# CIAM-Group/ComputerVision_Codes

Measured on AMD Instinct MI355X. Metric: frames/sec spatial-extract + per-video TCN latency, Cholec80, 1/2/4/8 GPU, higher is better.
Workload: dtype bf16

## Files before the change

computervision_codes_amd/csrc/bottleneck_fused.hip:

```cpp
#include "mt4_common.h"

typedef __bf16 bf16x8_t __attribute__((ext_vector_type(8)));

namespace {

constexpr int TH = 8, TW = 14, NHALO = 160, NPX = 128;
constexpr int ROW_B = 128;
constexpr int XS_BYTES = NHALO * ROW_B;
constexpr int T2_BYTES = NPX * ROW_B;
constexpr int T1_BYTES = XS_BYTES + 2 * ROW_B;
constexpr int YS_BYTES = NPX * 256;

struct BneckK {
    const char* x;
    char* y;
    const char *w1, *w2, *w3, *wds;
    const float *b1, *b2, *b3, *bds;
    int B, H, W, tiles_h, tiles_w;
    int nt;
    char* y2;
    const char* wn;
    const float* bn;
    int H2, W2;
};

__device__ __forceinline__ f32x4 bias4(const float* b, int n) {
    const float4 t = *(const float4*)(b + n);
    return (f32x4){t.x, t.y, t.z, t.w};
}

__device__ __forceinline__ uint2 relu_pack4(f32x4 v) {
    uint2 o = make_uint2(pack_bf16x2(v[0], v[1]), pack_bf16x2(v[2], v[3]));
    asm("v_pk_max_i16 %0, %0, 0" : "+v"(o.x));
    asm("v_pk_max_i16 %0, %0, 0" : "+v"(o.y));
    return o;
}

__device__ __forceinline__ f32x4 mfma_bf16(uint4 wfrag, uint4 xfrag, f32x4 acc) {
    return __builtin_amdgcn_mfma_f32_16x16x32_bf16(__builtin_bit_cast(bf16x8_t, wfrag), __builtin_bit_cast(bf16x8_t, xfrag), acc, 0, 0, 0);
}

template <int CIN, bool DS, bool NEXT = false>
__global__ __launch_bounds__(256, 2) void bottleneck64_fused_kernel(const BneckK a) {
    static_assert(!NEXT || !DS, "the following conv rides behind an identity block");
    constexpr int KC = CIN / 64;
    constexpr int NXS = KC > 1 ? 2 : 1;
    static_assert(DS ? CIN == 64 : CIN == 256, "layer1.0 (64 channels in, downsample branch) or layer1.1+ (256 in, identity)");
    extern __shared__ __attribute__((aligned(16))) char smem[];
    char* const xs = smem;
    char* const t2 = smem + NXS * XS_BYTES;
    char* const t1 = t2 + T2_BYTES;
    char* const ys = DS ? t1 : xs;

    const int tid = threadIdx.x;
    const int lane = tid & 63, wave = tid >> 6;
    const int r16 = lane & 15, q = lane >> 4;

    int bid = blockIdx.x;
    {
        const int nb = gridDim.x;
        const int q8 = nb >> 3, r8 = nb & 7;
        const int xcd = bid & 7, local = bid >> 3;
        bid = (xcd < r8 ? xcd * (q8 + 1) : r8 * (q8 + 1) + (xcd - r8) * q8) + local;
    }
    const int tpi = a.tiles_h * a.tiles_w;
    const int img = bid / tpi;
    const int trem = bid - img * tpi;
    const int th = trem / a.tiles_w;
    const int h0 = th * TH, w0 = (trem - th * a.tiles_w) * TW;
    const char* const ximg = a.x + (long long)img * a.H * a.W * (CIN * 2);
    char* const yimg = NEXT ? a.y + (long long)img * a.H2 * a.W2 * 512 : a.y + (long long)img * a.H * a.W * 512;

    const int ld_row = tid >> 3, ld_chunk = tid & 7;
    int xoff[5];
#pragma unroll
    for (int i = 0; i < 5; ++i) {
        const int hp = ld_row + 32 * i;
        const int h = h0 - 1 + (hp >> 4), w = w0 - 1 + (hp & 15);
        xoff[i] = ((unsigned)h < (unsigned)a.H && (unsigned)w < (unsigned)a.W) ? (h * a.W + w) * (CIN * 2) + ld_chunk * 16 : -1;
    }
    auto load_chunk = [&](int kc, uint4 (&stg)[5]) {
#pragma unroll
        for (int i = 0; i < 5; ++i) {
            stg[i] = make_uint4(0, 0, 0, 0);
            if (xoff[i] >= 0) stg[i] = *(const uint4*)(ximg + xoff[i] + kc * 128);
        }
    };
    auto store_chunk = [&](int buf, const uint4 (&stg)[5]) {
#pragma unroll
        for (int i = 0; i < 5; ++i) {
            const int hp = ld_row + 32 * i;
            *(uint4*)(xs + buf * XS_BYTES + hp * ROW_B + ((ld_chunk ^ (hp & 7)) << 4)) = stg[i];
        }
    };
    uint4 stg0[5], stg1[5];
    load_chunk(0, stg0);
    if constexpr (KC > 1) load_chunk(1, stg1);

    const int ch1 = wave * 16;
    uint4 wf1[KC * 2];
    {
        const char* wr = a.w1 + (wave * (KC * 2) * 64 + lane) * 16;
#pragma unroll
        for (int s = 0; s < KC * 2; ++s) wf1[s] = *(const uint4*)(wr + s * 1024);
    }
    f32x4 acc1[10];
    {
        const f32x4 b4 = bias4(a.b1, ch1 + q * 4);
#pragma unroll
        for (int i = 0; i < 10; ++i) acc1[i] = b4;
    }
    const int sw0 = (q ^ (r16 & 7)) << 4, sw1 = ((4 + q) ^ (r16 & 7)) << 4;
    uint2 res[DS ? 1 : 4][DS ? 1 : 8];
    const int res_off = (r16 + 1) * ROW_B + (((2 * wave + (q >> 1)) ^ ((r16 + 1) & 7)) << 4) + (q & 1) * 8;
#pragma unroll
    for (int kc = 0; kc < KC; ++kc) {
        if (kc & 1) store_chunk(1, stg1); else store_chunk(0, stg0);
        if (kc + 2 < KC) { if (kc & 1) load_chunk(kc + 2, stg1); else load_chunk(kc + 2, stg0); }
        __syncthreads();
        const char* sb = xs + (kc & 1) * XS_BYTES + r16 * ROW_B;
        uint4 fx[2][10];
#pragma unroll
        for (int kk = 0; kk < 2; ++kk)
#pragma unroll
            for (int i = 0; i < 10; ++i) fx[kk][i] = *(const uint4*)(sb + i * 16 * ROW_B + (kk ? sw1 : sw0));
        if constexpr (!DS) {
#pragma unroll
            for (int j = 0; j < 8; ++j) res[kc][j] = *(const uint2*)(xs + (kc & 1) * XS_BYTES + (j + 1) * (16 * ROW_B) + res_off);
        }
        asm volatile("" ::: "memory");
#pragma unroll
        for (int kk = 0; kk < 2; ++kk)
#pragma unroll
            for (int i = 0; i < 10; ++i) acc1[i] = mfma_bf16(wf1[kc * 2 + kk], fx[kk][i], acc1[i]);
    }
    uint4 wf2[18];
    {
        const char* wr = a.w2 + (wave * 18 * 64 + lane) * 16;
#pragma unroll
        for (int s = 0; s < 18; ++s) wf2[s] = *(const uint4*)(wr + s * 1024);
    }
    const int cb1 = (ch1 + q * 4) * 2;
    {
        const int wr_off = r16 * ROW_B + (((cb1 >> 4) ^ (r16 & 7)) << 4) + (cb1 & 8);
        const int w = w0 - 1 + r16;
#pragma unroll
        for (int i = 0; i < 10; ++i) {
            const int h = h0 - 1 + i;
            const bool in = (unsigned)h < (unsigned)a.H && (unsigned)w < (unsigned)a.W;
            uint2 o = make_uint2(0, 0);
            if (in) o = relu_pack4(acc1[i]);
            *(uint2*)(t1 + i * (16 * ROW_B) + wr_off) = o;
        }
    }
    __syncthreads();

    f32x4 acc2[8];
    {
        const f32x4 b4 = bias4(a.b2, ch1 + q * 4);
#pragma unroll
        for (int j = 0; j < 8; ++j) acc2[j] = b4;
    }
    int toff[3][2];
#pragma unroll
    for (int kw = 0; kw < 3; ++kw)
#pragma unroll
        for (int kk = 0; kk < 2; ++kk) toff[kw][kk] = (r16 + kw) * ROW_B + (((kk * 4 + q) ^ ((r16 + kw) & 7)) << 4);
#pragma unroll
    for (int hr = 0; hr < 10; ++hr) {
        uint4 fr[3][2];
#pragma unroll
        for (int kw = 0; kw < 3; ++kw)
#pragma unroll
            for (int kk = 0; kk < 2; ++kk) fr[kw][kk] = *(const uint4*)(t1 + hr * (16 * ROW_B) + toff[kw][kk]);
        asm volatile("" ::: "memory");
#pragma unroll
        for (int kh = 0; kh < 3; ++kh) {
            const int ty = hr - kh;
            if (ty >= 0 && ty < 8) {
#pragma unroll
                for (int kw = 0; kw < 3; ++kw)
#pragma unroll
                    for (int kk = 0; kk < 2; ++kk) acc2[ty] = mfma_bf16(wf2[(kh * 3 + kw) * 2 + kk], fr[kw][kk], acc2[ty]);
            }
        }
    }
    uint4 wf3[4][2];
    uint4 wfd[DS ? 4 : 1][2];
#pragma unroll
    for (int i = 0; i < 4; ++i) {
        const char* wr = a.w3 + ((4 * i + wave) * 2 * 64 + lane) * 16;
        wf3[i][0] = *(const uint4*)wr;
        wf3[i][1] = *(const uint4*)(wr + 1024);
        if constexpr (DS) {
            const char* wd = a.wds + ((4 * i + wave) * 2 * 64 + lane) * 16;
            wfd[i][0] = *(const uint4*)wd;
            wfd[i][1] = *(const uint4*)(wd + 1024);
        }
    }
    {
        const int wr_off = r16 * ROW_B + (((cb1 >> 4) ^ (r16 & 7)) << 4) + (cb1 & 8);
#pragma unroll
        for (int j = 0; j < 8; ++j) {
            const uint2 o = relu_pack4(acc2[j]);
            *(uint2*)(t2 + j * (16 * ROW_B) + wr_off) = o;
        }
    }
    __syncthreads();

    uint4 fx3[8][2];
#pragma unroll
    for (int j = 0; j < 8; ++j) {
        fx3[j][0] = *(const uint4*)(t2 + j * (16 * ROW_B) + r16 * ROW_B + sw0);
        fx3[j][1] = *(const uint4*)(t2 + j * (16 * ROW_B) + r16 * ROW_B + sw1);
    }
    const int st_tx = tid >> 4, st_chunk = tid & 15;
    uint4 wfn[NEXT ? 2 : 1][NEXT ? 8 : 1];
#pragma unroll
    for (int pass = 0; pass < 2; ++pass) {
        char* const ysp = NEXT ? xs + pass * YS_BYTES : ys;
        if (pass && !NEXT) __syncthreads();
#pragma unroll
        for (int ii = 0; ii < 2; ++ii) {
            const int i = pass * 2 + ii;
            const int ct = 4 * i + wave;
            f32x4 acc3[8];
            {
                const f32x4 b4 = bias4(a.b3, ct * 16 + q * 4);
#pragma unroll
                for (int j = 0; j < 8; ++j) acc3[j] = b4;
            }
#pragma unroll
            for (int kk = 0; kk < 2; ++kk)
#pragma unroll
                for (int j = 0; j < 8; ++j) acc3[j] = mfma_bf16(wf3[i][kk], fx3[j][kk], acc3[j]);
            if constexpr (DS) {
                const f32x4 bd4 = bias4(a.bds, ct * 16 + q * 4);
#pragma unroll
                for (int j = 0; j < 8; ++j) {
                    f32x4 accd = bd4;
#pragma unroll
                    for (int kk = 0; kk < 2; ++kk) accd = mfma_bf16(wfd[i][kk], *(const uint4*)(xs + (j + 1) * (16 * ROW_B) + toff[1][kk]), accd);
#pragma unroll
                    for (int e = 0; e < 4; ++e) acc3[j][e] += bf16_to_f32(f32_to_bf16(accd[e]));
                }
            } else {
#pragma unroll
                for (int j = 0; j < 8; ++j) {
                    acc3[j][0] += __uint_as_float(res[i][j].x << 16);
                    acc3[j][1] += __uint_as_float(res[i][j].x & 0xffff0000u);
                    acc3[j][2] += __uint_as_float(res[i][j].y << 16);
                    acc3[j][3] += __uint_as_float(res[i][j].y & 0xffff0000u);
                }
            }
            const int cbyte = ((ct - 8 * pass) * 16 + q * 4) * 2;
            const int wr_off = r16 * 256 + (((cbyte >> 4) ^ r16) << 4) + (cbyte & 8);
#pragma unroll
            for (int j = 0; j < 8; ++j) {
                const uint2 o = relu_pack4(acc3[j]);
                *(uint2*)(ysp + j * (16 * 256) + wr_off) = o;
            }
        }
        if constexpr (NEXT) {
            if (pass == 1) {
#pragma unroll
                for (int c = 0; c < 2; ++c)
#pragma unroll
                    for (int ks = 0; ks < 8; ++ks) wfn[c][ks] = *(const uint4*)(a.wn + (((2 * wave + c) * 8 + ks) * 64 + lane) * 16);
            }
        }
        __syncthreads();
        {
            const int w = w0 + st_tx;
            const int rd_off = st_tx * 256 + ((st_chunk ^ st_tx) << 4);
            if constexpr (NEXT) {
                if (st_tx < TW && w < a.W && !(st_tx & 1)) {
                    const uint4 v0 = *(const uint4*)(ysp + rd_off), v1 = *(const uint4*)(ysp + 2 * (16 * 256) + rd_off);
                    const uint4 v2 = *(const uint4*)(ysp + 4 * (16 * 256) + rd_off), v3 = *(const uint4*)(ysp + 6 * (16 * 256) + rd_off);
                    char* const yp = yimg + (unsigned)(((h0 >> 1) * a.W2 + (w >> 1)) * 512 + pass * 256 + st_chunk * 16);
                    const int rows = a.H - h0;
                    *(uint4*)yp = v0;
                    if (rows > 2) *(uint4*)(yp + a.W2 * 512) = v1;
                    if (rows > 4) *(uint4*)(yp + 2 * a.W2 * 512) = v2;
                    if (rows > 6) *(uint4*)(yp + 3 * a.W2 * 512) = v3;
                }
            } else if (st_tx < TW && w < a.W) {
                uint4 v[8];
#pragma unroll
                for (int ty = 0; ty < 8; ++ty) v[ty] = *(const uint4*)(ysp + ty * (16 * 256) + rd_off);
                asm volatile("" ::: "memory");
#pragma unroll
                for (int ty = 0; ty < 8; ++ty) {
                    if (h0 + ty < a.H) {
                        typedef unsigned u32x4 __attribute__((ext_vector_type(4)));
                        char* yp = yimg + (unsigned)((h0 + ty) * a.W * 512) + (unsigned)(w * 512 + pass * 256 + st_chunk * 16);
                        if (a.nt) __builtin_nontemporal_store((u32x4){v[ty].x, v[ty].y, v[ty].z, v[ty].w}, (u32x4*)yp);
                        else *(uint4*)yp = v[ty];
                    }
                }
            }
        }
    }
    if constexpr (NEXT) {
        f32x4 acc4[2][8];
#pragma unroll
        for (int c = 0; c < 2; ++c) {
            const f32x4 b4 = bias4(a.bn, (2 * wave + c) * 16 + q * 4);
#pragma unroll
            for (int j = 0; j < 8; ++j) acc4[c][j] = b4;
        }
#pragma unroll
        for (int ks = 0; ks < 8; ++ks) {
            uint4 fy[8];
            const char* yb = xs + (ks >> 2) * YS_BYTES + r16 * 256 + ((((ks & 3) * 4 + q) ^ r16) << 4);
#pragma unroll
            for (int j = 0; j < 8; ++j) fy[j] = *(const uint4*)(yb + j * (16 * 256));
            asm volatile("" ::: "memory");
#pragma unroll
            for (int c = 0; c < 2; ++c)
#pragma unroll
                for (int j = 0; j < 8; ++j) acc4[c][j] = mfma_bf16(wfn[c][ks], fy[j], acc4[c][j]);
        }
        __syncthreads();
#pragma unroll
        for (int c = 0; c < 2; ++c) {
            const int cbyte = ((2 * wave + c) * 16 + q * 4) * 2;
            const int wr_off = r16 * 256 + (((cbyte >> 4) ^ r16) << 4) + (cbyte & 8);
#pragma unroll
            for (int j = 0; j < 8; ++j) *(uint2*)(xs + j * (16 * 256) + wr_off) = relu_pack4(acc4[c][j]);
        }
        __syncthreads();
        const int w = w0 + st_tx;
        if (st_tx < TW && w < a.W) {
            const int rd_off = st_tx * 256 + ((st_chunk ^ st_tx) << 4);
            char* const y2img = a.y2 + (long long)img * a.H * a.W * 256;
            uint4 v[8];
#pragma unroll
            for (int ty = 0; ty < 8; ++ty) v[ty] = *(const uint4*)(xs + ty * (16 * 256) + rd_off);
            asm volatile("" ::: "memory");
#pragma unroll
            for (int ty = 0; ty < 8; ++ty) {
                if (h0 + ty < a.H) {
                    typedef unsigned u32x4 __attribute__((ext_vector_type(4)));
                    char* yp = y2img + (unsigned)(((h0 + ty) * a.W + w) * 256 + st_chunk * 16);
                    if (a.nt) __builtin_nontemporal_store((u32x4){v[ty].x, v[ty].y, v[ty].z, v[ty].w}, (u32x4*)yp);
                    else *(uint4*)yp = v[ty];
                }
            }
        }
    }
}

template <int CIN, bool DS, bool NEXT = false>
int launch(const BneckK& a, hipStream_t stream) {
    constexpr int NXS = CIN > 64 ? 2 : 1;
    constexpr int LDS = NXS * XS_BYTES + T2_BYTES + (DS ? YS_BYTES : T1_BYTES);
    static_assert(LDS <= 80 * 1024, "two workgroups per CU");
    static_assert(!NEXT || LDS >= 2 * YS_BYTES, "both output passes stay in LDS");
    auto fn = bottleneck64_fused_kernel<CIN, DS, NEXT>;
    MT4_RAISE_LDS(fn);
    const long long nblk = (long long)a.B * a.tiles_h * a.tiles_w;
    hipLaunchKernelGGL(fn, dim3((unsigned)nblk), dim3(256), LDS, stream, a);
    return mt4_check_launch();
}

}

__global__ void bneck_pack_kernel(const u16* __restrict__ w, uint4* __restrict__ out, int ctiles, int ksteps, int row_elems) {
    const int i = blockIdx.x * blockDim.x + threadIdx.x;
    if (i >= ctiles * ksteps * 64) return;
    const int lane = i & 63, fs = i >> 6;
    const int step = fs % ksteps, tile = fs / ksteps;
    out[i] = *(const uint4*)(w + (long long)(tile * 16 + (lane & 15)) * row_elems + step * 32 + (lane >> 4) * 8);
}

static inline long long bneck_frag_bytes(int Cin, bool ds) { return ((long long)4 * (Cin / 32) + 4 * 18 + 16 * 2 + (ds ? 16 * (Cin / 32) : 0)) * 1024; }

extern "C" int64_t mt4_bottleneck_packed_bytes(int32_t Cin, int32_t has_downsample) {
    if (!((has_downsample && Cin == 64) || (!has_downsample && Cin == 256))) return MT4_EUNSUPPORTED;
    return bneck_frag_bytes(Cin, has_downsample != 0);
}

extern "C" int mt4_bottleneck_pack_bf16(const void* w1, const void* w2, const void* w3, const void* wds, int32_t Cin, void* out, void* stream) {
    mt4_clear_error();
    if (!w1 || !w2 || !w3 || !out) return MT4_EINVAL;
    if (!((wds && Cin == 64) || (!wds && Cin == 256))) return MT4_EUNSUPPORTED;
    if (((uintptr_t)w1 | (uintptr_t)w2 | (uintptr_t)w3 | (uintptr_t)wds | (uintptr_t)out) & 15) return MT4_EALIGN;
    hipStream_t s = (hipStream_t)stream;
    const int k1 = Cin / 32;
    char* o = (char*)out;
    const int r1 = (int)mt4_conv_packed_k(Cin, 1, 1, MT4_BF16), r2 = (int)mt4_conv_packed_k(64, 3, 3, MT4_BF16), r3 = (int)mt4_conv_packed_k(64, 1, 1, MT4_BF16);
    auto go = [&](const void* w, int ctiles, int ksteps, int row_elems) {
        const int n = ctiles * ksteps * 64;
        hipLaunchKernelGGL(bneck_pack_kernel, dim3((n + 255) / 256), dim3(256), 0, s, (const u16*)w, (uint4*)o, ctiles, ksteps, row_elems);
        o += (long long)n * 16;
    };
    go(w1, 4, k1, r1);
    go(w2, 4, 18, r2);
    go(w3, 16, 2, r3);
    if (wds) go(wds, 16, k1, r1);
    return mt4_check_launch();
}

extern "C" int mt4_bottleneck_fused_bf16(const void* x, void* y, const void* w_frag, const float* b1, const float* b2, const float* b3, const float* bds,
                                         int32_t B, int32_t H, int32_t W, int32_t Cin, int32_t mid, void* stream) {
    mt4_clear_error();
    if (!x || !y || !w_frag || !b1 || !b2 || !b3 || B <= 0 || H <= 0 || W <= 0) return MT4_EINVAL;
    const bool ds = bds != nullptr;
    if (mid != 64 || !((ds && Cin == 64) || (!ds && Cin == 256))) return MT4_EUNSUPPORTED;
    if (((uintptr_t)x | (uintptr_t)y | (uintptr_t)w_frag | (uintptr_t)b1 | (uintptr_t)b2 | (uintptr_t)b3 | (uintptr_t)bds) & 15) return MT4_EALIGN;
    if ((long long)H * W * 512 > 0x7fffffffLL) return MT4_EUNSUPPORTED;
    BneckK a;
    a.x = (const char*)x; a.y = (char*)y;
    const int k1 = Cin / 32;
    a.w1 = (const char*)w_frag;
    a.w2 = a.w1 + (long long)4 * k1 * 1024;
    a.w3 = a.w2 + (long long)4 * 18 * 1024;
    a.wds = ds ? a.w3 + (long long)16 * 2 * 1024 : nullptr;
    a.b1 = b1; a.b2 = b2; a.b3 = b3; a.bds = bds;
    a.B = B; a.H = H; a.W = W;
    a.tiles_h = cdiv(H, TH); a.tiles_w = cdiv(W, TW);
    a.nt = 1;
    if ((long long)B * a.tiles_h * a.tiles_w > 0x7fffffffLL) return MT4_EUNSUPPORTED;
    return ds ? launch<64, true>(a, (hipStream_t)stream) : launch<256, false>(a, (hipStream_t)stream);
}

extern "C" int64_t mt4_bottleneck_next_packed_bytes(void) { return (int64_t)8 * 8 * 1024; }

extern "C" int mt4_bottleneck_pack_next_bf16(const void* w1_next, void* out, void* stream) {
    mt4_clear_error();
    if (!w1_next || !out) return MT4_EINVAL;
    if (((uintptr_t)w1_next | (uintptr_t)out) & 15) return MT4_EALIGN;
    const int n = 8 * 8 * 64;
    hipLaunchKernelGGL(bneck_pack_kernel, dim3((n + 255) / 256), dim3(256), 0, (hipStream_t)stream, (const u16*)w1_next, (uint4*)out, 8, 8,
                       (int)mt4_conv_packed_k(256, 1, 1, MT4_BF16));
    return mt4_check_launch();
}

extern "C" int mt4_bottleneck_fused_next_bf16(const void* x, void* y_even, void* t_next, const void* w_frag, const float* b1, const float* b2,
                                              const float* b3, const void* w_next, const float* b_next, int32_t B, int32_t H, int32_t W, void* stream) {
    mt4_clear_error();
    if (!x || !y_even || !t_next || !w_frag || !b1 || !b2 || !b3 || !w_next || !b_next || B <= 0 || H <= 0 || W <= 0) return MT4_EINVAL;
    if (((uintptr_t)x | (uintptr_t)y_even | (uintptr_t)t_next | (uintptr_t)w_frag | (uintptr_t)b1 | (uintptr_t)b2 | (uintptr_t)b3 | (uintptr_t)w_next |
         (uintptr_t)b_next) & 15)
        return MT4_EALIGN;
    if ((long long)H * W * 512 > 0x7fffffffLL) return MT4_EUNSUPPORTED;
    BneckK a{};
    a.x = (const char*)x; a.y = (char*)y_even; a.y2 = (char*)t_next;
    a.w1 = (const char*)w_frag;
    a.w2 = a.w1 + (long long)4 * 8 * 1024;
    a.w3 = a.w2 + (long long)4 * 18 * 1024;
    a.wds = nullptr;
    a.b1 = b1; a.b2 = b2; a.b3 = b3; a.bds = nullptr;
    a.wn = (const char*)w_next; a.bn = b_next;
    a.B = B; a.H = H; a.W = W; a.H2 = (H + 1) / 2; a.W2 = (W + 1) / 2;
    a.tiles_h = cdiv(H, TH); a.tiles_w = cdiv(W, TW);
    a.nt = 1;
    if ((long long)B * a.tiles_h * a.tiles_w > 0x7fffffffLL) return MT4_EUNSUPPORTED;
    return launch<256, false, true>(a, (hipStream_t)stream);
}

extern "C" int mt4_pack_fragments_bf16(const void* w_packed, int32_t rows, int32_t row_elems, void* out, void* stream) {
    mt4_clear_error();
    if (!w_packed || !out || rows <= 0 || row_elems <= 0) return MT4_EINVAL;
    if ((rows % 16) || (row_elems % 32)) return MT4_EUNSUPPORTED;
    if (((uintptr_t)w_packed | (uintptr_t)out) & 15) return MT4_EALIGN;
    const long long n = (long long)(rows / 16) * (row_elems / 32) * 64;
    if (n > 0x7fffffffLL) return MT4_EUNSUPPORTED;
    hipLaunchKernelGGL(bneck_pack_kernel, dim3((unsigned)((n + 255) / 256)), dim3(256), 0, (hipStream_t)stream, (const u16*)w_packed, (uint4*)out, rows / 16,
                       row_elems / 32, row_elems);
    return mt4_check_launch();
}
```

computervision_codes_amd/csrc/igemm_conv.hip:

```cpp
#include "mt4_common.h"
#include <cstdlib>

typedef __bf16 bf16x8_t __attribute__((ext_vector_type(8)));
typedef unsigned v4u __attribute__((ext_vector_type(4)));

__device__ __forceinline__ v4u make_srd(const void* p, unsigned bytes) {
    const unsigned long long u = (unsigned long long)p;
    v4u r;
    r.x = __builtin_amdgcn_readfirstlane((unsigned)u);
    r.y = __builtin_amdgcn_readfirstlane((unsigned)(u >> 32) & 0xffffu);
    r.z = __builtin_amdgcn_readfirstlane(bytes);
    r.w = 0x00020000u;
    return r;
}

template <int N, int STRIDE>
__device__ __forceinline__ void lds_dma16_group(v4u srd, const unsigned (&voff)[N], unsigned soff, unsigned lds_addr) {
    unsigned keep;
    if constexpr (N == 1) {
        asm volatile("s_mov_b32 %0, m0\n\ts_mov_b32 m0, %4\n\ts_nop 0\n\tbuffer_load_dwordx4 %1, %2, %3 offen lds\n\ts_mov_b32 m0, %0"
                     : "=&s"(keep) : "v"(voff[0]), "s"(srd), "s"(soff), "s"(lds_addr) : "memory");
    } else if constexpr (N == 2) {
        asm volatile("s_mov_b32 %0, m0\n\ts_mov_b32 m0, %5\n\ts_nop 0\n\tbuffer_load_dwordx4 %1, %3, %4 offen lds\n\t"
                     "s_add_u32 m0, m0, %6\n\ts_nop 0\n\tbuffer_load_dwordx4 %2, %3, %4 offen lds\n\ts_mov_b32 m0, %0"
                     : "=&s"(keep) : "v"(voff[0]), "v"(voff[1]), "s"(srd), "s"(soff), "s"(lds_addr), "n"(STRIDE) : "memory", "scc");
    } else {
        static_assert(N == 4, "1, 2 or 4 pieces");
        asm volatile("s_mov_b32 %0, m0\n\ts_mov_b32 m0, %7\n\ts_nop 0\n\tbuffer_load_dwordx4 %1, %5, %6 offen lds\n\t"
                     "s_add_u32 m0, m0, %8\n\ts_nop 0\n\tbuffer_load_dwordx4 %2, %5, %6 offen lds\n\t"
                     "s_add_u32 m0, m0, %8\n\ts_nop 0\n\tbuffer_load_dwordx4 %3, %5, %6 offen lds\n\t"
                     "s_add_u32 m0, m0, %8\n\ts_nop 0\n\tbuffer_load_dwordx4 %4, %5, %6 offen lds\n\ts_mov_b32 m0, %0"
                     : "=&s"(keep) : "v"(voff[0]), "v"(voff[1]), "v"(voff[2]), "v"(voff[3]), "s"(srd), "s"(soff), "s"(lds_addr),
                       "n"(STRIDE)
                     : "memory", "scc");
    }
}

__device__ __forceinline__ void lds_dma16(v4u srd, unsigned voff, unsigned lds_addr) {
    unsigned keep;
    asm volatile(
        "s_mov_b32 %0, m0\n\t"
        "s_mov_b32 m0, %3\n\t"
        "s_nop 0\n\t"
        "buffer_load_dwordx4 %1, %2, 0 offen lds\n\t"
        "s_mov_b32 m0, %0"
        : "=&s"(keep)
        : "v"(voff), "s"(srd), "s"(lds_addr)
        : "memory");
}

struct ConvK {
    const char* x;
    const char* w;
    const float* bias;
    const char* res;
    char* y;
    const int* row_map;
    int map_len;
    int map_img;
    int y_ld, res_ld;
    int res_f32;
    int B, H, W, Cin, Ho, Wo, Cout, KH, KW, sh, sw, ph, pw, dh, dw, relu;
    int M, HoWo, CPT, SPT, taps, nsteps, n_tiles, total_tiles;
    long long x_img_bytes;
    int pix_bytes;
    unsigned x_bytes, w_bytes;
    long long x_total_bytes;
    unsigned x_bias;
    int w_row_bytes;
    int nt_epi;
    const char* x2;
    long long x2_img_bytes, x2_total_bytes;
    int x2_W, x2_s, x2_pix_bytes, x2_HoWo, x2_Wo;
    int nsteps1;
    double* stat_sums;
    const char* f_w;
    const float* f_bias;
    char* f_y;
    int f_cout, f_relu, f_w_row_bytes;
};

template <int TPR, int NTH, int CH, int BN>
__device__ __forceinline__ void colstat_flush(double (&cs)[CH], double (&cq)[CH], char* smem, double* __restrict__ sums, int n0, int Cout, int tid) {
    static_assert(TPR <= 64 && 64 % TPR == 0, "a wave covers whole rows of the read-back");
    constexpr int NW = NTH / 64;
    const int lane = tid & 63, wave = tid >> 6;
#pragma unroll
    for (int o = TPR; o < 64; o <<= 1) {
#pragma unroll
        for (int e = 0; e < CH; ++e) { cs[e] += __shfl_xor(cs[e], o); cq[e] += __shfl_xor(cq[e], o); }
    }
    double* red = (double*)smem;
    __syncthreads();
    if (lane < TPR) {
#pragma unroll
        for (int e = 0; e < CH; ++e) {
            red[(wave * 2) * BN + lane * CH + e] = cs[e];
            red[(wave * 2 + 1) * BN + lane * CH + e] = cq[e];
        }
    }
    __syncthreads();
    for (int col = tid; col < 2 * BN; col += NTH) {
        const int h = col / BN, c = col - h * BN;
        double t = 0.0;
#pragma unroll
        for (int w = 0; w < NW; ++w) t += red[(w * 2 + h) * BN + c];
        if (n0 + c < Cout) atomicAdd(sums + (long long)h * Cout + n0 + c, t);
    }
}

template <typename T, int BM, int BN, int WAVES_M, int WAVES_N, int STAGES, bool FAST, bool OUT_F32, int KS = 1, bool DUAL = false, bool STATS = false>
__global__ __launch_bounds__(WAVES_M * WAVES_N * KS * 64) void igemm_conv_kernel(const ConvK a) {
    static_assert(!DUAL || (FAST && sizeof(T) == 2 && KS == 1), "the second K source exists on the bf16 LDS-DMA path");
    static_assert(!STATS || (KS == 1 && !DUAL && WAVES_M * WAVES_N * BN * 16 <= (BM + BN) * 128), "channel sums: one-group forms whose LDS holds the waves' partial rows");
    constexpr int ES = (int)sizeof(T);
    constexpr int ROWS = BM + BN;
    constexpr int NWG = WAVES_M * WAVES_N;
    constexpr int NW = NWG * KS;
    constexpr int NTH = NW * 64;
    constexpr int GTH = NWG * 64;
    constexpr int RPP = GTH / 8;
    static_assert(KS == 1 || FAST, "K-split groups exist on the LDS-DMA path only");
    constexpr int NLD = ROWS / RPP;
    constexpr int NLD_X = BM / RPP;
    constexpr int NLD_W = BN / RPP;
    constexpr int WM = BM / WAVES_M, WN = BN / WAVES_N;
    constexpr int MT = WM / 16, NT = WN / 16;
    constexpr int STAGE_BYTES = ROWS * 128;
    static_assert(NW == 4 || NW == 8 || NW == 16, "4, 8 or 16 waves");
    static_assert(BM % RPP == 0 && BN % RPP == 0 && WM % 16 == 0 && WN % 16 == 0, "tile shape");
    extern __shared__ __attribute__((aligned(16))) char smem[];

    const int tid = threadIdx.x;
    const int lane = tid & 63, wave = tid >> 6;
    const int grp = KS > 1 ? wave / NWG : 0;
    const int wave_l = KS > 1 ? wave % NWG : wave;
    const int tid_l = KS > 1 ? tid % GTH : tid;
    const int wave_m = wave_l / WAVES_N, wave_n = wave_l % WAVES_N;
    const int r16 = lane & 15, q = lane >> 4;

    int bid = blockIdx.x;
    {
        const int nb = gridDim.x;
        const int q8 = nb >> 3, r8 = nb & 7;
        const int xcd = bid & 7, local = bid >> 3;
        bid = (xcd < r8 ? xcd * (q8 + 1) : r8 * (q8 + 1) + (xcd - r8) * q8) + local;
    }
    const int tile_m = bid / a.n_tiles;
    const int tile_n = bid - tile_m * a.n_tiles;
    const int m0 = tile_m * BM, n0 = tile_n * BN;

    const int ld_row = tid_l >> 3, ld_chunk = tid_l & 7;
    const int st_off = ld_row * 128 + ((ld_chunk ^ (ld_row & 7)) << 4);

    f32x4 acc[NT][MT];
#pragma unroll
    for (int i = 0; i < NT; ++i) {
        const int n = n0 + wave_n * WN + i * 16 + q * 4;
        f32x4 b4 = (f32x4){0.f, 0.f, 0.f, 0.f};
        if (a.bias && grp == 0) {
            if ((a.Cout & 3) == 0) {
                if (n < a.Cout) { const float4 t = *(const float4*)(a.bias + n); b4 = (f32x4){t.x, t.y, t.z, t.w}; }
            } else {
#pragma unroll
                for (int e = 0; e < 4; ++e) if (n + e < a.Cout) b4[e] = a.bias[n + e];
            }
        }
#pragma unroll
        for (int j = 0; j < MT; ++j) acc[i][j] = b4;
    }

    const int rd_x = (wave_m * WM + r16) * 128;
    const int rd_w = (BM + wave_n * WN + r16) * 128;
    const int nsteps = a.nsteps;

    auto compute = [&](const char* sb) {
#pragma unroll
        for (int kk = 0; kk < 2; ++kk) {
            const int sw_off = ((kk * 4 + q) ^ (r16 & 7)) << 4;
            uint4 fx[MT], fw[NT];
#pragma unroll
            for (int j = 0; j < MT; ++j) fx[j] = *(const uint4*)(sb + rd_x + j * 16 * 128 + sw_off);
#pragma unroll
            for (int i = 0; i < NT; ++i) fw[i] = *(const uint4*)(sb + rd_w + i * 16 * 128 + sw_off);
#pragma unroll
            for (int i = 0; i < NT; ++i)
#pragma unroll
                for (int j = 0; j < MT; ++j) {
                    if constexpr (sizeof(T) == 2) {
                        acc[i][j] = __builtin_amdgcn_mfma_f32_16x16x32_bf16(
                            __builtin_bit_cast(bf16x8_t, fw[i]), __builtin_bit_cast(bf16x8_t, fx[j]), acc[i][j], 0, 0, 0);
                    } else {
                        acc[i][j] = __builtin_amdgcn_mfma_f32_16x16x4f32(__uint_as_float(fw[i].x), __uint_as_float(fx[j].x),
                                                                         acc[i][j], 0, 0, 0);
                        acc[i][j] = __builtin_amdgcn_mfma_f32_16x16x4f32(__uint_as_float(fw[i].y), __uint_as_float(fx[j].y),
                                                                         acc[i][j], 0, 0, 0);
                        acc[i][j] = __builtin_amdgcn_mfma_f32_16x16x4f32(__uint_as_float(fw[i].z), __uint_as_float(fx[j].z),
                                                                         acc[i][j], 0, 0, 0);
                        acc[i][j] = __builtin_amdgcn_mfma_f32_16x16x4f32(__uint_as_float(fw[i].w), __uint_as_float(fx[j].w),
                                                                         acc[i][j], 0, 0, 0);
                    }
                }
        }
    };

    if constexpr (FAST) {
        const long long org = (long long)(m0 / a.HoWo) * a.x_img_bytes;
        const long long left = a.x_total_bytes - org + a.x_bias;
        const v4u rsx = make_srd(a.x - a.x_bias + org, (unsigned)(left < 0x7fffffffLL ? left : 0x7fffffffLL));
        const v4u rsw = make_srd(a.w, a.w_bytes);
        constexpr unsigned OOB = 0x80000000u;
        const int gch = ld_chunk ^ (ld_row & 7);
        const int wave_u = __builtin_amdgcn_readfirstlane(wave_l);
        const int grp_u = __builtin_amdgcn_readfirstlane(grp);
        char* const smem_g = smem + grp_u * (STAGES * STAGE_BYTES);
        const unsigned lds_base = (unsigned)(uintptr_t)(__attribute__((address_space(3))) char*)smem_g;
        int xoff[NLD_X];
        unsigned hmask = 0, wmask = 0;
        static_assert(NLD_X <= 4, "one mask byte per staged pixel row");
#pragma unroll
        for (int i = 0; i < NLD_X; ++i) {
            const int m = m0 + ld_row + RPP * i;
            const bool ok = m < a.M;
            const int mm = ok ? m : 0;
            int hi0 = 0, wi0 = 0;
            long long base;
            if (a.HoWo == 1) {
                hi0 = -a.ph;
                wi0 = -a.pw;
                base = (long long)mm * a.x_img_bytes + (long long)(hi0 * a.W + wi0) * a.pix_bytes;
            } else {
                const int b = mm / a.HoWo;
                const int rem = mm - b * a.HoWo;
                const int ho = rem / a.Wo;
                const int wo = rem - ho * a.Wo;
                hi0 = ho * a.sh - a.ph;
                wi0 = wo * a.sw - a.pw;
                base = (long long)b * a.x_img_bytes + (long long)(hi0 * a.W + wi0) * a.pix_bytes;
            }
            xoff[i] = (int)(base - org) + gch * 16 + (int)a.x_bias;
            if (ok) {
                for (int kh = 0; kh < a.KH; ++kh)
                    if ((unsigned)(hi0 + kh * a.dh) < (unsigned)a.H) hmask |= 1u << (8 * i + kh);
                for (int kw = 0; kw < a.KW; ++kw)
                    if ((unsigned)(wi0 + kw * a.dw) < (unsigned)a.W) wmask |= 1u << (8 * i + kw);
            }
        }
        unsigned woff[NLD_W];
#pragma unroll
        for (int i = 0; i < NLD_W; ++i) {
            const int n = n0 + ld_row + RPP * i;
            woff[i] = n < a.Cout ? (unsigned)(n * a.w_row_bytes + gch * 16) : OOB;
        }
        unsigned xoff2[DUAL ? NLD_X : 1];
        v4u rsx2 = rsx;
        if constexpr (DUAL) {
            const long long org2 = (long long)(m0 / a.x2_HoWo) * a.x2_img_bytes;
            const long long left2 = a.x2_total_bytes - org2;
            rsx2 = make_srd(a.x2 + org2, (unsigned)(left2 < 0x7fffffffLL ? left2 : 0x7fffffffLL));
#pragma unroll
            for (int i = 0; i < NLD_X; ++i) {
                const int m = m0 + ld_row + RPP * i;
                const int mm = m < a.M ? m : 0;
                const int b = mm / a.x2_HoWo;
                const int rem = mm - b * a.x2_HoWo;
                const int ho = rem / a.x2_Wo;
                const int wo = rem - ho * a.x2_Wo;
                const long long base2 = (long long)b * a.x2_img_bytes + (long long)(ho * a.x2_s * a.x2_W + wo * a.x2_s) * a.x2_pix_bytes;
                xoff2[i] = m < a.M ? (unsigned)((int)(base2 - org2) + gch * 16) : OOB;
            }
        }
        int f_kh = 0, f_kw = 0, f_cs = 0;
        auto issue = [&](int step, int stage) {
            if constexpr (DUAL) {
                if (step >= a.nsteps1) {
                    const unsigned dst2 = lds_base + stage * STAGE_BYTES + wave_u * 1024;
                    lds_dma16_group<NLD_X, RPP * 128>(rsx2, xoff2, (unsigned)__builtin_amdgcn_readfirstlane((step - a.nsteps1) * 128), dst2);
                    lds_dma16_group<NLD_W, RPP * 128>(rsw, woff, (unsigned)__builtin_amdgcn_readfirstlane(step * 128), dst2 + BM * 128);
                    return;
                }
            }
            const int delta = (f_kh * a.dh * a.W + f_kw * a.dw) * a.pix_bytes + f_cs * 128;
            const unsigned bits = (hmask >> f_kh) & (wmask >> f_kw);
            const int wstep = (f_kh * a.KW + f_kw) * a.SPT + f_cs;
#pragma unroll
            for (int adv = 0; adv < KS; ++adv) {
                if (++f_kw == a.KW) {
                    f_kw = 0;
                    if (++f_kh == a.KH) { f_kh = 0; ++f_cs; }
                }
            }
            f_cs = __builtin_amdgcn_readfirstlane(f_cs);
            f_kw = __builtin_amdgcn_readfirstlane(f_kw);
            f_kh = __builtin_amdgcn_readfirstlane(f_kh);
            const unsigned dst = lds_base + stage * STAGE_BYTES + wave_u * 1024;
            unsigned vx[NLD_X];
#pragma unroll
            for (int i = 0; i < NLD_X; ++i) vx[i] = ((bits >> (8 * i)) & 1u) ? (unsigned)xoff[i] : OOB;
            lds_dma16_group<NLD_X, RPP * 128>(rsx, vx, (unsigned)__builtin_amdgcn_readfirstlane(delta), dst);
            lds_dma16_group<NLD_W, RPP * 128>(rsw, woff, (unsigned)__builtin_amdgcn_readfirstlane(wstep * 128), dst + BM * 128);
        };
        auto wait_keep = [&](int groups) {
            if (groups <= 0) asm volatile("s_waitcnt vmcnt(0)" ::: "memory");
            else if (groups == 1) asm volatile("s_waitcnt vmcnt(%0)" ::"n"(NLD) : "memory");
            else asm volatile("s_waitcnt vmcnt(%0)" ::"n"(2 * NLD) : "memory");
        };
        static_assert(STAGES >= 2 && STAGES <= 4 && (STAGES - 2) * NLD <= 63, "wait_keep covers up to 2 groups in flight");
        int my_steps = nsteps, iters = nsteps;
        if constexpr (KS > 1) {
            my_steps = (nsteps - grp_u + KS - 1) / KS;
            iters = (nsteps + KS - 1) / KS;
            for (int adv = 0; adv < grp_u; ++adv) {
                if (++f_kw == a.KW) {
                    f_kw = 0;
                    if (++f_kh == a.KH) { f_kh = 0; ++f_cs; }
                }
            }
        }
#pragma unroll
        for (int s0 = 0; s0 < STAGES - 1; ++s0)
            if (s0 < my_steps) issue(s0, s0);
        wait_keep((my_steps < STAGES - 1 ? my_steps : STAGES - 1) - 1);
        __syncthreads();
        int cur = 0, fill = STAGES - 1;
        for (int step = 0; step < iters; ++step) {
            if (step + STAGES - 1 < my_steps) issue(step + STAGES - 1, fill);
            if (KS == 1 || step < my_steps) compute(smem_g + cur * STAGE_BYTES);
            const int rem = my_steps - 1 - step;
            wait_keep((rem < STAGES - 1 ? rem : STAGES - 1) - 1);
            __syncthreads();
            cur = cur + 1 == STAGES ? 0 : cur + 1;
            fill = fill + 1 == STAGES ? 0 : fill + 1;
        }
        if constexpr (KS > 1) {
            f32x4* red = (f32x4*)smem;
            if (grp > 0) {
#pragma unroll
                for (int i = 0; i < NT; ++i)
#pragma unroll
                    for (int j = 0; j < MT; ++j) red[(((grp - 1) * NWG + wave_l) * (NT * MT) + i * MT + j) * 64 + lane] = acc[i][j];
            }
            __syncthreads();
            if (grp == 0) {
#pragma unroll
                for (int g = 1; g < KS; ++g)
#pragma unroll
                    for (int i = 0; i < NT; ++i)
#pragma unroll
                        for (int j = 0; j < MT; ++j) acc[i][j] += red[(((g - 1) * NWG + wave_l) * (NT * MT) + i * MT + j) * 64 + lane];
            }
            __syncthreads();
        }
    } else {
        const char* px_base[NLD_X];
        int px_hi0[NLD_X], px_wi0[NLD_X];
        bool px_ok[NLD_X];
#pragma unroll
        for (int i = 0; i < NLD_X; ++i) {
            const int m = m0 + ld_row + RPP * i;
            px_ok[i] = m < a.M;
            const int mm = px_ok[i] ? m : 0;
            const int b = mm / a.HoWo;
            const int rem = mm - b * a.HoWo;
            const int ho = rem / a.Wo;
            const int wo = rem - ho * a.Wo;
            px_hi0[i] = ho * a.sh - a.ph;
            px_wi0[i] = wo * a.sw - a.pw;
            px_base[i] = a.x + (long long)b * a.x_img_bytes;
        }
        const char* w_ptr[NLD_W];
        bool w_ok[NLD_W];
#pragma unroll
        for (int i = 0; i < NLD_W; ++i) {
            const int n = n0 + ld_row + RPP * i;
            w_ok[i] = n < a.Cout;
            w_ptr[i] = a.w + (long long)(w_ok[i] ? n : 0) * a.w_row_bytes + ld_chunk * 16;
        }
        uint4 stg[NLD];
        auto load_step = [&](int step) {
            const int g = step * 8 + ld_chunk;
            const int tap = g / a.CPT;
            const int cc = g - tap * a.CPT;
            const int kh = tap / a.KW;
            const int kw = tap - kh * a.KW;
            const int choff = cc * 16;
            const bool tap_ok = tap < a.taps;
            const int dhi = kh * a.dh, dwi = kw * a.dw;
#pragma unroll
            for (int i = 0; i < NLD_X; ++i) {
                const int hi = px_hi0[i] + dhi, wi = px_wi0[i] + dwi;
                const bool ok = tap_ok && px_ok[i] && (unsigned)hi < (unsigned)a.H && (unsigned)wi < (unsigned)a.W;
                uint4 v = make_uint4(0, 0, 0, 0);
                if (ok) v = *(const uint4*)(px_base[i] + (long long)(hi * a.W + wi) * a.pix_bytes + choff);
                stg[i] = v;
            }
#pragma unroll
            for (int i = 0; i < NLD_W; ++i) {
                uint4 v = make_uint4(0, 0, 0, 0);
                if (w_ok[i]) v = *(const uint4*)(w_ptr[i] + (long long)step * 128);
                stg[NLD_X + i] = v;
            }
        };
        auto store_stage = [&](int stage) {
            char* base = smem + stage * STAGE_BYTES + st_off;
#pragma unroll
            for (int i = 0; i < NLD; ++i) *(uint4*)(base + i * RPP * 128) = stg[i];
        };
        load_step(0);
        store_stage(0);
        __syncthreads();
        for (int step = 0; step < nsteps; ++step) {
            const int cur = step & 1;
            const bool more = step + 1 < nsteps;
            if (more) load_step(step + 1);
            compute(smem + cur * STAGE_BYTES);
            if (more) store_stage(cur ^ 1);
            __syncthreads();
        }
    }

    constexpr int OS = OUT_F32 ? 4 : 2;
    constexpr int CH = 16 / OS;
    constexpr int ROWB = BN * 4 + 16;
    constexpr int PASSES = (BM * ROWB > 4 * STAGE_BYTES) ? 4 : (BM * ROWB > 2 * STAGE_BYTES) ? 2 : 1;
    static_assert(BM / PASSES * ROWB <= 2 * STAGE_BYTES, "epilogue staging fits the main-loop LDS");
    static_assert(MT % PASSES == 0, "passes split the m-tiles of a wave");
    constexpr int MTP = MT / PASSES;
    constexpr int WMP = WM / PASSES;
    constexpr int BMP = BM / PASSES;
    constexpr int TPR = BN / CH;
    constexpr int RPI = NTH / TPR;
    constexpr int ITERS = (BMP + RPI - 1) / RPI;
    constexpr int RB = (sizeof(T) == 2 && CH == 4) ? 8 : 16;
    constexpr bool MIXED = sizeof(T) == 2 && OUT_F32;
    if ((a.Cout % CH) == 0) {
        const int rc = tid % TPR, rr = tid / TPR;
        const int n = n0 + rc * CH;
        double cs[STATS ? CH : 1], cq[STATS ? CH : 1];
        if constexpr (STATS) {
#pragma unroll
            for (int e = 0; e < CH; ++e) cs[e] = cq[e] = 0.0;
        }
#pragma unroll
        for (int p = 0; p < PASSES; ++p) {
            long long orow[ITERS];
            uint4 rres[ITERS];
#pragma unroll
            for (int it = 0; it < ITERS; ++it) {
                const int lrow = rr + it * RPI;
                const int trow = (lrow / WMP) * WM + p * WMP + (lrow % WMP);
                int m = m0 + trow;
                orow[it] = -1;
                rres[it] = make_uint4(0, 0, 0, 0);
                if (lrow < BMP && m < a.M && n < a.Cout) {
                    if (a.row_map) m = (m / a.map_len) * a.map_img + a.row_map[m % a.map_len];
                    orow[it] = m;
                    if (a.res) {
                        const char* rp = a.res + ((long long)m * a.res_ld + n) * ES;
                        if (MIXED && a.res_f32) rres[it] = *(const uint4*)(a.res + ((long long)m * a.res_ld + n) * 4);
                        else if constexpr (RB == 16) {
                            typedef unsigned u32x4 __attribute__((ext_vector_type(4)));
                            if (a.nt_epi) { const u32x4 t = __builtin_nontemporal_load((const u32x4*)rp); rres[it] = make_uint4(t.x, t.y, t.z, t.w); }
                            else rres[it] = *(const uint4*)rp;
                        }
                        else { const uint2 r2 = *(const uint2*)rp; rres[it] = make_uint4(r2.x, r2.y, 0, 0); }
                    }
                }
            }
            if (p) __syncthreads();
            if (KS == 1 || grp == 0) {
#pragma unroll
                for (int jj = 0; jj < MTP; ++jj) {
                    const int lrow = wave_m * WMP + jj * 16 + r16;
#pragma unroll
                    for (int i = 0; i < NT; ++i) {
                        const int nl = wave_n * WN + i * 16 + q * 4;
                        *(f32x4*)(smem + lrow * ROWB + nl * 4) = acc[i][p * MTP + jj];
                    }
                }
            }
            __syncthreads();
#pragma unroll
            for (int it = 0; it < ITERS; ++it) {
                if (orow[it] < 0) continue;
                const int lrow = rr + it * RPI;
                float v[CH];
                *(float4*)&v[0] = *(const float4*)(smem + lrow * ROWB + rc * CH * 4);
                if constexpr (CH == 8) *(float4*)&v[4] = *(const float4*)(smem + lrow * ROWB + rc * CH * 4 + 16);
                const long long o = orow[it] * a.y_ld + n;
                if (a.res && a.relu == 3) {
                    const uint4 rv = rres[it];
                    if (MIXED && a.res_f32) {
                        if (!(__uint_as_float(rv.x) > 0.f)) v[0] = 0.f;
                        if (!(__uint_as_float(rv.y) > 0.f)) v[1] = 0.f;
                        if (!(__uint_as_float(rv.z) > 0.f)) v[2] = 0.f;
                        if (!(__uint_as_float(rv.w) > 0.f)) v[3] = 0.f;
                    } else if constexpr (sizeof(T) == 2) {
                        const uint32_t u[4] = {rv.x, rv.y, rv.z, rv.w};
#pragma unroll
                        for (int e = 0; e < CH / 2; ++e) {
                            if (!(__uint_as_float(u[e] << 16) > 0.f)) v[2 * e] = 0.f;
                            if (!(__uint_as_float(u[e] & 0xffff0000u) > 0.f)) v[2 * e + 1] = 0.f;
                        }
                    } else {
                        if (!(__uint_as_float(rv.x) > 0.f)) v[0] = 0.f;
                        if (!(__uint_as_float(rv.y) > 0.f)) v[1] = 0.f;
                        if (!(__uint_as_float(rv.z) > 0.f)) v[2] = 0.f;
                        if (!(__uint_as_float(rv.w) > 0.f)) v[3] = 0.f;
                    }
                } else if (a.res) {
                    const uint4 rv = rres[it];
                    if (MIXED && a.res_f32) {
                        v[0] += __uint_as_float(rv.x); v[1] += __uint_as_float(rv.y);
                        v[2] += __uint_as_float(rv.z); v[3] += __uint_as_float(rv.w);
                    } else if constexpr (sizeof(T) == 2) {
                        const uint32_t u[4] = {rv.x, rv.y, rv.z, rv.w};
#pragma unroll
                        for (int e = 0; e < CH / 2; ++e) {
                            v[2 * e] += __uint_as_float(u[e] << 16);
                            v[2 * e + 1] += __uint_as_float(u[e] & 0xffff0000u);
                        }
                    } else {
                        v[0] += __uint_as_float(rv.x); v[1] += __uint_as_float(rv.y);
                        v[2] += __uint_as_float(rv.z); v[3] += __uint_as_float(rv.w);
                    }
                }
                if (a.relu == 1) {
#pragma unroll
                    for (int e = 0; e < CH; ++e) v[e] = fmaxf(v[e], 0.f);
                } else if (a.relu == 2) {
                    gelu_erf_n(v);
                }
                if constexpr (OUT_F32) {
                    *(float4*)(a.y + o * 4) = make_float4(v[0], v[1], v[2], v[3]);
                    if constexpr (STATS) {
#pragma unroll
                        for (int e = 0; e < 4; ++e) { const double dv = (double)v[e]; cs[e] += dv; cq[e] = fma(dv, dv, cq[e]); }
                    }
                } else {
                    typedef unsigned u32x4 __attribute__((ext_vector_type(4)));
                    const u32x4 ov = {pack_bf16x2(v[0], v[1]), pack_bf16x2(v[2], v[3]), pack_bf16x2(v[4], v[5]), pack_bf16x2(v[6], v[7])};
                    if (a.nt_epi) __builtin_nontemporal_store(ov, (u32x4*)(a.y + o * 2));
                    else *(uint4*)(a.y + o * 2) = make_uint4(ov.x, ov.y, ov.z, ov.w);
                    if constexpr (STATS) {
#pragma unroll
                        for (int e = 0; e < 4; ++e) {
                            const double lo = (double)__uint_as_float(ov[e] << 16), hi = (double)__uint_as_float(ov[e] & 0xffff0000u);
                            cs[2 * e] += lo; cq[2 * e] = fma(lo, lo, cq[2 * e]); cs[2 * e + 1] += hi; cq[2 * e + 1] = fma(hi, hi, cq[2 * e + 1]);
                        }
                    }
                }
            }
        }
        if constexpr (STATS)
            colstat_flush<TPR, NTH, CH, BN>(cs, cq, smem, a.stat_sums + (long long)(tile_m & (MT4_STAT_REPLICAS - 1)) * 2 * a.Cout, n0, a.Cout, tid);
        return;
    }
    if (KS > 1 && grp != 0) return;
#pragma unroll
    for (int j = 0; j < MT; ++j) {
        int m = m0 + wave_m * WM + j * 16 + r16;
        if (m >= a.M) continue;
        if (a.row_map) m = (m / a.map_len) * a.map_img + a.row_map[m % a.map_len];
#pragma unroll
        for (int i = 0; i < NT; ++i) {
            const int n = n0 + wave_n * WN + i * 16 + q * 4;
            if (n >= a.Cout) continue;
            const f32x4 v = acc[i][j];
            const long long o = (long long)m * a.y_ld + n;
            const long long ro = (long long)m * a.res_ld + n;
#pragma unroll
            for (int e = 0; e < 4; ++e) {
                if (n + e >= a.Cout) break;
                float f = v[e];
                if (a.res) {
                    float rvv;
                    if ((sizeof(T) == 2 && OUT_F32) && a.res_f32) rvv = *(const float*)(a.res + (ro + e) * 4);
                    else if constexpr (sizeof(T) == 2) rvv = bf16_to_f32(*(const u16*)(a.res + (ro + e) * 2));
                    else rvv = *(const float*)(a.res + (ro + e) * 4);
                    if (a.relu == 3) f = rvv > 0.f ? f : 0.f;
                    else f += rvv;
                }
                if (a.relu == 1) f = fmaxf(f, 0.f);
                else if (a.relu == 2) f = gelu_erf(f);
                if constexpr (OUT_F32) *(float*)(a.y + (o + e) * 4) = f;
                else *(u16*)(a.y + (o + e) * 2) = f32_to_bf16(f);
            }
        }
    }
}

template <int BM, int BN, int WAVES_M, int WAVES_N, int WS, bool EXPAND = false, bool STATS = false>
__global__ __launch_bounds__(WAVES_M * WAVES_N * 64, WAVES_M * WAVES_N == 4 ? 2 : 1) void conv3x3_patch_kernel(const ConvK a, const int pra, const int npatch) {
    static_assert(!EXPAND || BN == 128, "the expansion needs a pixel's whole channel vector in the tile");
    static_assert(!(EXPAND && STATS), "the expansion form takes no statistics");
    constexpr int NW = WAVES_M * WAVES_N;
    constexpr int NTH = NW * 64;
    constexpr int RPP = NTH / 8;
    constexpr int NLD_W = BN >= RPP ? BN / RPP : 1;
    constexpr int WM = BM / WAVES_M, WN = BN / WAVES_N;
    constexpr int MT = WM / 16, NT = WN / 16;
    constexpr int WSTAGE = BN * 128;
    static_assert((BN % RPP == 0 || RPP % BN == 0) && WM % 16 == 0 && WN % 16 == 0 && MT <= 4, "tile shape");
    static_assert((WS >= 2 && WS <= 4) || WS == 9, "weight ring depth (9: all taps of a single-slice layer resident, no barrier in the K loop)");
    constexpr bool RESIDENT = WS == 9;
    extern __shared__ __attribute__((aligned(16))) char smem[];

    const int tid = threadIdx.x;
    const int lane = tid & 63, wave = tid >> 6;
    const int wave_m = wave / WAVES_N, wave_n = wave % WAVES_N;
    const int r16 = lane & 15, q = lane >> 4;
    int bid = blockIdx.x;
    {
        const int nb = gridDim.x;
        const int q8 = nb >> 3, r8 = nb & 7;
        const int xcd = bid & 7, local = bid >> 3;
        bid = (xcd < r8 ? xcd * (q8 + 1) : r8 * (q8 + 1) + (xcd - r8) * q8) + local;
    }
    const int tile_m = bid / a.n_tiles;
    const int tile_n = bid - tile_m * a.n_tiles;
    const int m0 = tile_m * BM, n0 = tile_n * BN;
    const int ld_row = tid >> 3, ld_chunk = tid & 7;

    f32x4 acc[NT][MT];
#pragma unroll
    for (int i = 0; i < NT; ++i) {
        const int n = n0 + wave_n * WN + i * 16 + q * 4;
        f32x4 b4 = (f32x4){0.f, 0.f, 0.f, 0.f};
        if (a.bias && n < a.Cout) { const float4 t = *(const float4*)(a.bias + n); b4 = (f32x4){t.x, t.y, t.z, t.w}; }
#pragma unroll
        for (int j = 0; j < MT; ++j) acc[i][j] = b4;
    }

    int vm[MT];
#pragma unroll
    for (int j = 0; j < MT; ++j) {
        int m = m0 + wave_m * WM + j * 16 + r16;
        m = m < a.M ? m : a.M - 1;
        const int rem = m % a.HoWo;
        const int ho = rem / a.W;
        const int wo = rem - ho * a.W;
        const int wv = (wo > 0 ? 1 : 0) | 2 | (wo < a.W - 1 ? 4 : 0);
        vm[j] = (ho > 0 ? wv : 0) | (wv << 3) | (ho < a.H - 1 ? wv << 6 : 0);
    }

    const int zr = BM + 2 * a.W + 2;
    const int shift = (a.W + 1) * a.pix_bytes;
    const v4u rsx = make_srd(a.x - shift, a.x_bytes + (unsigned)shift);
    const v4u rsw = make_srd(a.w, a.w_bytes);
    constexpr unsigned OOB = 0x80000000u;
    const int gch = ld_chunk ^ (ld_row & 7);
    const int wave_u = __builtin_amdgcn_readfirstlane(wave);
    const unsigned lds_base = (unsigned)(uintptr_t)(__attribute__((address_space(3))) char*)smem;
    const int patch_bytes = pra * 128;
    const unsigned w_base = lds_base + npatch * patch_bytes;
    const int npp = (pra + RPP - 1) / RPP;
    unsigned woff[NLD_W];
#pragma unroll
    for (int i = 0; i < NLD_W; ++i) {
        const int n = n0 + ld_row + RPP * i;
        woff[i] = n < a.Cout ? (unsigned)(n * a.w_row_bytes + gch * 16) : OOB;
    }
    auto issue_patch = [&](int piece, int cs, int buf) {
        if (piece * RPP + wave_u * 8 < pra) {
            const int p = m0 + piece * RPP + ld_row;
            const unsigned v[1] = {(p >= a.W + 1 && piece * RPP + ld_row < zr) ? (unsigned)(p * a.pix_bytes + gch * 16) : OOB};
            lds_dma16_group<1, 0>(rsx, v, (unsigned)__builtin_amdgcn_readfirstlane(cs * 128),
                                  lds_base + buf * patch_bytes + piece * (RPP * 128) + wave_u * 1024);
        }
    };
    auto issue_w = [&](int wstep, int stage) {
        if (BN >= RPP || wave_u * 8 < BN)
        lds_dma16_group<NLD_W, RPP * 128>(rsw, woff, (unsigned)__builtin_amdgcn_readfirstlane(wstep * 128), w_base + stage * WSTAGE + wave_u * 1024);
    };
    const int rd_w = (wave_n * WN + r16) * 128;
    auto compute = [&](const char* pb, const char* wb, int toff, int tap) {
        const int prow = wave_m * WM + r16 + toff;
        const int tbit = 1 << tap;
        const char* xr[MT];
#pragma unroll
        for (int j = 0; j < MT; ++j) xr[j] = pb + ((vm[j] & tbit) ? prow + j * 16 : zr + ((prow ^ zr) & 1)) * 128;
#pragma unroll
        for (int kk = 0; kk < 2; ++kk) {
            const int swx = ((kk * 4 + q) ^ (prow & 7)) << 4;
            const int sww = ((kk * 4 + q) ^ (r16 & 7)) << 4;
            uint4 fx[MT], fw[NT];
#pragma unroll
            for (int j = 0; j < MT; ++j) fx[j] = *(const uint4*)(xr[j] + swx);
#pragma unroll
            for (int i = 0; i < NT; ++i) fw[i] = *(const uint4*)(wb + rd_w + i * 16 * 128 + sww);
#pragma unroll
            for (int i = 0; i < NT; ++i)
#pragma unroll
                for (int j = 0; j < MT; ++j)
                    acc[i][j] = __builtin_amdgcn_mfma_f32_16x16x32_bf16(__builtin_bit_cast(bf16x8_t, fw[i]), __builtin_bit_cast(bf16x8_t, fx[j]),
                                                                        acc[i][j], 0, 0, 0);
        }
    };

    const int SPT = a.SPT;
    const int nsteps = 9 * SPT;
    int i_tap = 0, i_cs = 0, i_stage = 0;
    auto issue_next_w = [&]() {
        issue_w(i_tap * SPT + i_cs, i_stage);
        if (++i_tap == 9) { i_tap = 0; ++i_cs; }
        i_stage = i_stage + 1 == WS ? 0 : i_stage + 1;
    };
    auto wait_allowed = [&](int n) {
        switch (n) {
            case 0: asm volatile("s_waitcnt vmcnt(0)" ::: "memory"); break;
            case 1: asm volatile("s_waitcnt vmcnt(1)" ::: "memory"); break;
            case 2: asm volatile("s_waitcnt vmcnt(2)" ::: "memory"); break;
            case 3: asm volatile("s_waitcnt vmcnt(3)" ::: "memory"); break;
            case 4: asm volatile("s_waitcnt vmcnt(4)" ::: "memory"); break;
            case 5: asm volatile("s_waitcnt vmcnt(5)" ::: "memory"); break;
            default: asm volatile("s_waitcnt vmcnt(6)" ::: "memory"); break;
        }
    };
    static_assert(RESIDENT || (WS - 2) * (NLD_W + 1) <= 6, "wait_allowed covers up to 6 instructions in flight");
    for (int piece = 0; piece < npp; ++piece) issue_patch(piece, 0, 0);
#pragma unroll
    for (int s0 = 0; s0 < (RESIDENT ? 9 : WS - 1); ++s0)
        if (s0 < nsteps) issue_next_w();
    asm volatile("s_waitcnt vmcnt(0)" ::: "memory");
    __syncthreads();
    int step = 0, cur = 0;
    int c_prev = 0;
#pragma unroll 1
    for (int cs = 0; cs < SPT; ++cs) {
        const char* pb = smem + (cs & (npatch - 1)) * patch_bytes;
        int kh = 0, kw = 0;
#pragma unroll 1
        for (int tap = 0; tap < 9; ++tap, ++step) {
            int c_now = 0;
            if constexpr (!RESIDENT) {
                if (step + WS - 1 < nsteps) { issue_next_w(); c_now = NLD_W; }
                if (cs + 1 < SPT && tap < npp && tap * RPP + wave_u * 8 < pra) { issue_patch(tap, cs + 1, (cs + 1) & 1); ++c_now; }
            }
            compute(pb, smem + npatch * patch_bytes + cur * WSTAGE, kh * a.W + kw, tap);
            if (++kw == 3) { kw = 0; ++kh; }
            cur = cur + 1 == WS ? 0 : cur + 1;
            if constexpr (!RESIDENT) {
                c_now = __builtin_amdgcn_readfirstlane(c_now);
                wait_allowed(WS == 2 ? 0 : WS == 3 ? c_now : c_now + c_prev);
                c_prev = c_now;
                __syncthreads();
            }
        }
    }
    if constexpr (RESIDENT) __syncthreads();

    constexpr int ROWB = BN * 4 + 16;
    constexpr int PASSES = BN >= 256 ? 4 : 2;
    static_assert(MT % PASSES == 0, "passes split the m-tiles of a wave");
    constexpr int MTP = MT / PASSES, WMP = WM / PASSES, BMP = BM / PASSES;
    constexpr int TPR = BN / 8, RPI = NTH / TPR;
    constexpr int ITERS = (BMP + RPI - 1) / RPI;
    const int rc = tid % TPR, rr = tid / TPR;
    const int n = n0 + rc * 8;
    typedef unsigned u32x4 __attribute__((ext_vector_type(4)));
    if constexpr (EXPAND) {
        char* const t2p = smem;
        char* const stg = smem + 2 * BM * 128;
#pragma unroll
        for (int j = 0; j < MT; ++j) {
            const int row = wave_m * WM + j * 16 + r16;
#pragma unroll
            for (int i = 0; i < NT; ++i) {
                const int ch = wave_n * WN + i * 16 + q * 4;
                const int cb = (ch & 63) * 2;
                f32x4 v = acc[i][j];
                if (a.relu == 1) {
#pragma unroll
                    for (int e = 0; e < 4; ++e) v[e] = fmaxf(v[e], 0.f);
                }
                *(uint2*)(t2p + (ch >> 6) * (BM * 128) + row * 128 + (((cb >> 4) ^ (row & 7)) << 4) + (cb & 8)) =
                    make_uint2(pack_bf16x2(v[0], v[1]), pack_bf16x2(v[2], v[3]));
            }
        }
        __syncthreads();
        const int nchunk = a.f_cout >> 7;
        auto load_res = [&](int c, int p, u32x4 (&r)[ITERS]) {
            const int n2 = c * 128 + rc * 8;
#pragma unroll
            for (int it = 0; it < ITERS; ++it) {
                const int lrow = rr + it * RPI;
                const int m = m0 + (lrow / WMP) * WM + p * WMP + (lrow % WMP);
                r[it] = (u32x4){0u, 0u, 0u, 0u};
                if (a.res && lrow < BMP && m < a.M) {
                    const u32x4* rp = (const u32x4*)(a.res + ((long long)m * a.f_cout + n2) * 2);
                    r[it] = a.nt_epi ? __builtin_nontemporal_load(rp) : *rp;
                }
            }
        };
        uint4 fa[NT][4];
        auto load_w = [&](int c) {
#pragma unroll
            for (int i = 0; i < NT; ++i)
#pragma unroll
                for (int ks = 0; ks < 4; ++ks) fa[i][ks] = *(const uint4*)(a.f_w + ((long long)(((c * 8 + wave_n * NT + i) * 4 + ks) * 64 + lane)) * 16);
        };
        static_assert(PASSES == 2, "the residual prefetch alternates between two register sets");
        u32x4 r0[ITERS], r1[ITERS];
        load_res(0, 0, r0);
        load_w(0);
#pragma unroll 1
        for (int c = 0; c < nchunk; ++c) {
            f32x4 acc2[NT][MT];
#pragma unroll
            for (int i = 0; i < NT; ++i) {
                const float4 t = *(const float4*)(a.f_bias + c * 128 + wave_n * WN + i * 16 + q * 4);
#pragma unroll
                for (int j = 0; j < MT; ++j) acc2[i][j] = (f32x4){t.x, t.y, t.z, t.w};
            }
#pragma unroll
            for (int ks = 0; ks < 4; ++ks) {
                uint4 fb[MT];
#pragma unroll
                for (int j = 0; j < MT; ++j) {
                    const int prow = wave_m * WM + j * 16 + r16;
                    fb[j] = *(const uint4*)(t2p + (ks >> 1) * (BM * 128) + prow * 128 + ((((ks & 1) * 4 + q) ^ (prow & 7)) << 4));
                }
#pragma unroll
                for (int i = 0; i < NT; ++i)
#pragma unroll
                    for (int j = 0; j < MT; ++j)
                        acc2[i][j] = __builtin_amdgcn_mfma_f32_16x16x32_bf16(__builtin_bit_cast(bf16x8_t, fa[i][ks]), __builtin_bit_cast(bf16x8_t, fb[j]),
                                                                             acc2[i][j], 0, 0, 0);
            }
            if (c + 1 < nchunk) load_w(c + 1);
            const int n2 = c * 128 + rc * 8;
#pragma unroll
            for (int p = 0; p < PASSES; ++p) {
                if (p == 0) load_res(c, 1, r1);
                else if (c + 1 < nchunk) load_res(c + 1, 0, r0);
                if (c || p) __syncthreads();
#pragma unroll
                for (int jj = 0; jj < MTP; ++jj) {
                    const int lrow = wave_m * WMP + jj * 16 + r16;
#pragma unroll
                    for (int i = 0; i < NT; ++i) *(f32x4*)(stg + lrow * ROWB + (wave_n * WN + i * 16 + q * 4) * 4) = acc2[i][p * MTP + jj];
                }
                __syncthreads();
#pragma unroll
                for (int it = 0; it < ITERS; ++it) {
                    const int lrow = rr + it * RPI;
                    const int m = m0 + (lrow / WMP) * WM + p * WMP + (lrow % WMP);
                    if (lrow >= BMP || m >= a.M) continue;
                    float v[8];
                    *(float4*)&v[0] = *(const float4*)(stg + lrow * ROWB + rc * 32);
                    *(float4*)&v[4] = *(const float4*)(stg + lrow * ROWB + rc * 32 + 16);
                    if (a.res) {
                        const u32x4 rv = p ? r1[it] : r0[it];
#pragma unroll
                        for (int e = 0; e < 4; ++e) {
                            v[2 * e] += __uint_as_float(rv[e] << 16);
                            v[2 * e + 1] += __uint_as_float(rv[e] & 0xffff0000u);
                        }
                    }
                    if (a.f_relu) {
#pragma unroll
                        for (int e = 0; e < 8; ++e) v[e] = fmaxf(v[e], 0.f);
                    }
                    const u32x4 ov = {pack_bf16x2(v[0], v[1]), pack_bf16x2(v[2], v[3]), pack_bf16x2(v[4], v[5]), pack_bf16x2(v[6], v[7])};
                    char* yp = a.f_y + ((long long)m * a.f_cout + n2) * 2;
                    if (a.nt_epi) __builtin_nontemporal_store(ov, (u32x4*)yp);
                    else *(uint4*)yp = make_uint4(ov.x, ov.y, ov.z, ov.w);
                }
            }
        }
        return;
    }
    double cs[STATS ? 8 : 1], cq[STATS ? 8 : 1];
#pragma unroll
    for (int e = 0; e < (STATS ? 8 : 1); ++e) cs[e] = cq[e] = 0.0;
#pragma unroll
    for (int p = 0; p < PASSES; ++p) {
        u32x4 rres[ITERS];
#pragma unroll
        for (int it = 0; it < ITERS; ++it) {
            const int lrow = rr + it * RPI;
            const int m = m0 + (lrow / WMP) * WM + p * WMP + (lrow % WMP);
            rres[it] = (u32x4){0u, 0u, 0u, 0u};
            if (a.res && lrow < BMP && m < a.M && n < a.Cout) {
                const u32x4* rp = (const u32x4*)(a.res + ((long long)m * a.res_ld + n) * 2);
                rres[it] = a.nt_epi ? __builtin_nontemporal_load(rp) : *rp;
            }
        }
        if (p) __syncthreads();
#pragma unroll
        for (int jj = 0; jj < MTP; ++jj) {
            const int lrow = wave_m * WMP + jj * 16 + r16;
#pragma unroll
            for (int i = 0; i < NT; ++i) *(f32x4*)(smem + lrow * ROWB + (wave_n * WN + i * 16 + q * 4) * 4) = acc[i][p * MTP + jj];
        }
        __syncthreads();
#pragma unroll
        for (int it = 0; it < ITERS; ++it) {
            const int lrow = rr + it * RPI;
            const int m = m0 + (lrow / WMP) * WM + p * WMP + (lrow % WMP);
            if (lrow >= BMP || m >= a.M || n >= a.Cout) continue;
            float v[8];
            *(float4*)&v[0] = *(const float4*)(smem + lrow * ROWB + rc * 32);
            *(float4*)&v[4] = *(const float4*)(smem + lrow * ROWB + rc * 32 + 16);
            if (a.res) {
#pragma unroll
                for (int e = 0; e < 4; ++e) {
                    v[2 * e] += __uint_as_float(rres[it][e] << 16);
                    v[2 * e + 1] += __uint_as_float(rres[it][e] & 0xffff0000u);
                }
            }
            if (a.relu == 1) {
#pragma unroll
                for (int e = 0; e < 8; ++e) v[e] = fmaxf(v[e], 0.f);
            }
            const u32x4 ov = {pack_bf16x2(v[0], v[1]), pack_bf16x2(v[2], v[3]), pack_bf16x2(v[4], v[5]), pack_bf16x2(v[6], v[7])};
            char* yp = a.y + ((long long)m * a.y_ld + n) * 2;
            if (a.nt_epi) __builtin_nontemporal_store(ov, (u32x4*)yp);
            else *(uint4*)yp = make_uint4(ov.x, ov.y, ov.z, ov.w);
            if constexpr (STATS) {
#pragma unroll
                for (int e = 0; e < 4; ++e) {
                    const double lo = (double)__uint_as_float(ov[e] << 16), hi = (double)__uint_as_float(ov[e] & 0xffff0000u);
                    cs[2 * e] += lo; cq[2 * e] = fma(lo, lo, cq[2 * e]); cs[2 * e + 1] += hi; cq[2 * e + 1] = fma(hi, hi, cq[2 * e + 1]);
                }
            }
        }
    }
    if constexpr (STATS) colstat_flush<TPR, NTH, 8, BN>(cs, cq, smem, a.stat_sums + (long long)(tile_m & (MT4_STAT_REPLICAS - 1)) * 2 * a.Cout, n0, a.Cout, tid);
}

template <int BM, int WAVES_M, int WAVES_N>
__global__ __launch_bounds__(WAVES_M * WAVES_N * 64) __attribute__((amdgpu_waves_per_eu(6, 6))) void stem_patch_kernel(const ConvK a, const int pra) {
    constexpr int BN = 64;
    constexpr int NW = WAVES_M * WAVES_N;
    constexpr int NTH = NW * 64;
    constexpr int PPP = NTH * 16 / 32;
    constexpr int WM = BM / WAVES_M, WN = BN / WAVES_N;
    constexpr int MT = WM / 16, NT = WN / 16;
    static_assert(NW == 8 && WM % 16 == 0 && WN % 16 == 0 && MT <= 4, "tile shape (8 waves stage the 64 weight rows in one pass)");
    extern __shared__ __attribute__((aligned(16))) char smem[];

    const int tid = threadIdx.x;
    const int lane = tid & 63, wave = tid >> 6;
    const int wave_m = wave / WAVES_N, wave_n = wave % WAVES_N;
    const int r16 = lane & 15, q = lane >> 4;
    int bid = blockIdx.x;
    {
        const int nb = gridDim.x;
        const int q8 = nb >> 3, r8 = nb & 7;
        const int xcd = bid & 7, local = bid >> 3;
        bid = (xcd < r8 ? xcd * (q8 + 1) : r8 * (q8 + 1) + (xcd - r8) * q8) + local;
    }
    const int img = bid / a.n_tiles;
    const int m0 = img * a.HoWo + (bid - img * a.n_tiles) * BM;
    const int m_end = (img + 1) * a.HoWo;

    f32x4 acc[NT][MT];
#pragma unroll
    for (int i = 0; i < NT; ++i) {
        const int n = wave_n * WN + i * 16 + q * 4;
        f32x4 b4 = (f32x4){0.f, 0.f, 0.f, 0.f};
        if (a.bias && n < a.Cout) { const float4 t = *(const float4*)(a.bias + n); b4 = (f32x4){t.x, t.y, t.z, t.w}; }
#pragma unroll
        for (int j = 0; j < MT; ++j) acc[i][j] = b4;
    }

    auto frame_index = [&](int m) {
        const int b = m / a.HoWo;
        const int rem = m - b * a.HoWo;
        const int ho = rem / a.Wo;
        return (b * a.H + ho) * a.W + (rem - ho * a.Wo);
    };
    const int p0 = __builtin_amdgcn_readfirstlane(frame_index(m0));
    int base[MT];
#pragma unroll
    for (int j = 0; j < MT; ++j) {
        const int m = m0 + wave_m * WM + j * 16 + r16;
        base[j] = frame_index(m < m_end ? m : m_end - 1) - p0 + (q >> 1);
    }

    const v4u rsx = make_srd(a.x, a.x_bytes);
    const v4u rsw = make_srd(a.w, a.w_bytes);
    constexpr unsigned OOB = 0x80000000u;
    const int wave_u = __builtin_amdgcn_readfirstlane(wave);
    const unsigned lds_base = (unsigned)(uintptr_t)(__attribute__((address_space(3))) char*)smem;
    const int patch_bytes = pra * 32;
    {
        const int npp = (pra + PPP - 1) / PPP;
        for (int piece = 0; piece < npp; ++piece) {
            if (piece * PPP + wave_u * 32 < pra) {
                const int t = piece * PPP + (tid >> 1);
                const int h = tid & 1;
                const unsigned v[1] = {(unsigned)((p0 + t) * 32 + h * 16)};
                lds_dma16_group<1, 0>(rsx, v, 0u, lds_base + piece * (PPP * 32) + wave_u * 1024);
            }
        }
        const int ld_row = tid >> 3, ld_chunk = tid & 7;
        const int gch = ld_chunk ^ (ld_row & 7);
        const unsigned woff[1] = {ld_row < a.Cout ? (unsigned)(ld_row * a.w_row_bytes + gch * 16) : OOB};
        for (int kh = 0; kh < a.KH; ++kh)
            lds_dma16_group<1, 0>(rsw, woff, (unsigned)__builtin_amdgcn_readfirstlane(kh * 128), lds_base + patch_bytes + kh * (BN * 128) + wave_u * 1024);
    }
    asm volatile("s_waitcnt vmcnt(0)" ::: "memory");
    __syncthreads();

    const int rd_w = (wave_n * WN + r16) * 128;
#pragma unroll 1
    for (int kh = 0; kh < a.KH; ++kh) {
        const char* wb = smem + patch_bytes + kh * (BN * 128);
#pragma unroll
        for (int kk = 0; kk < 2; ++kk) {
            const int sww = ((kk * 4 + q) ^ (r16 & 7)) << 4;
            uint4 fx[MT], fw[NT];
#pragma unroll
            for (int j = 0; j < MT; ++j) {
                const int pix = base[j] + kh * a.W + kk * 2;
                fx[j] = *(const uint4*)(smem + pix * 32 + ((q & 1) << 4));
            }
#pragma unroll
            for (int i = 0; i < NT; ++i) fw[i] = *(const uint4*)(wb + rd_w + i * 16 * 128 + sww);
#pragma unroll
            for (int i = 0; i < NT; ++i)
#pragma unroll
                for (int j = 0; j < MT; ++j)
                    acc[i][j] = __builtin_amdgcn_mfma_f32_16x16x32_bf16(__builtin_bit_cast(bf16x8_t, fw[i]), __builtin_bit_cast(bf16x8_t, fx[j]),
                                                                        acc[i][j], 0, 0, 0);
        }
    }
    __syncthreads();

    constexpr int ROWB = BN * 4 + 16;
    constexpr int PASSES = 2;
    static_assert(MT % PASSES == 0, "passes split the m-tiles of a wave");
    constexpr int MTP = MT / PASSES, WMP = WM / PASSES, BMP = BM / PASSES;
    constexpr int TPR = BN / 8, RPI = NTH / TPR;
    constexpr int ITERS = (BMP + RPI - 1) / RPI;
    const int rc = tid % TPR, rr = tid / TPR;
    const int n = rc * 8;
#pragma unroll
    for (int p = 0; p < PASSES; ++p) {
        if (p) __syncthreads();
#pragma unroll
        for (int jj = 0; jj < MTP; ++jj) {
            const int lrow = wave_m * WMP + jj * 16 + r16;
#pragma unroll
            for (int i = 0; i < NT; ++i) *(f32x4*)(smem + lrow * ROWB + (wave_n * WN + i * 16 + q * 4) * 4) = acc[i][p * MTP + jj];
        }
        __syncthreads();
#pragma unroll
        for (int it = 0; it < ITERS; ++it) {
            const int lrow = rr + it * RPI;
            const int m = m0 + (lrow / WMP) * WM + p * WMP + (lrow % WMP);
            if (lrow >= BMP || m >= m_end || n >= a.Cout) continue;
            float v[8];
            *(float4*)&v[0] = *(const float4*)(smem + lrow * ROWB + rc * 32);
            *(float4*)&v[4] = *(const float4*)(smem + lrow * ROWB + rc * 32 + 16);
            if (a.relu == 1) {
#pragma unroll
                for (int e = 0; e < 8; ++e) v[e] = fmaxf(v[e], 0.f);
            }
            typedef unsigned u32x4 __attribute__((ext_vector_type(4)));
            const u32x4 ov = {pack_bf16x2(v[0], v[1]), pack_bf16x2(v[2], v[3]), pack_bf16x2(v[4], v[5]), pack_bf16x2(v[6], v[7])};
            char* yp = a.y + ((long long)m * a.y_ld + n) * 2;
            if (a.nt_epi) __builtin_nontemporal_store(ov, (u32x4*)yp);
            else *(uint4*)yp = make_uint4(ov.x, ov.y, ov.z, ov.w);
        }
    }
}

struct StemPoolK {
    const char* x;
    const char* w;
    const float* bias;
    char* y;
    unsigned x_bytes, w_bytes;
    int w_row_bytes, Cout, KH;
    int Hs, Ws, Ho, Wo, Hp, Wp;
    int tiles_per_img;
    int pra;
    int segs, cw, rs, wp_seg;
    int ctw;
};

template <int MT, int NPASS>
__global__ __launch_bounds__(512, 4) void stem_pool_kernel(const StemPoolK a) {
    constexpr int NT = 2, BN = 64, NTH = 512, PPP = NTH * 16 / 32;
    constexpr int MTP = (MT + NPASS - 1) / NPASS;
    extern __shared__ __attribute__((aligned(16))) char smem[];
    const int tid = threadIdx.x;
    const int lane = tid & 63, wave = tid >> 6;
    const int wave_m = wave >> 1, wave_n = wave & 1;
    const int r16 = lane & 15, q = lane >> 4;
    int bid = blockIdx.x;
    {
        const int nb = gridDim.x;
        const int q8 = nb >> 3, r8 = nb & 7;
        const int xcd = bid & 7, local = bid >> 3;
        bid = (xcd < r8 ? xcd * (q8 + 1) : r8 * (q8 + 1) + (xcd - r8) * q8) + local;
    }
    const int img = bid / a.tiles_per_img;
    const int trem = bid - img * a.tiles_per_img;
    const int rp = trem / a.segs;
    const int Q0 = (trem - rp * a.segs) * a.wp_seg;
    const int cs0 = max(2 * Q0 - 1, 0);
    const int P0 = rp * 2;
    const int c0 = 2 * P0 - 1;
    const int tpr = a.cw >> 4;
    const int ntile = 5 * tpr;

    f32x4 bias4v[NT];
#pragma unroll
    for (int i = 0; i < NT; ++i) {
        const int n = wave_n * 32 + i * 16 + q * 4;
        bias4v[i] = (f32x4){0.f, 0.f, 0.f, 0.f};
        if (a.bias && n < a.Cout) { const float4 t = *(const float4*)(a.bias + n); bias4v[i] = (f32x4){t.x, t.y, t.z, t.w}; }
    }
    const int p0 = __builtin_amdgcn_readfirstlane((img * a.Hs + c0) * a.Ws + cs0);
    int base[MT], trow[MT], tcol0[MT];
    const int lane_px = r16 + (q >> 1);
    const int wave_m_u = __builtin_amdgcn_readfirstlane(wave_m);
    const unsigned tpr_magic = 65536u / (unsigned)tpr + 1u;
#pragma unroll
    for (int j = 0; j < MT; ++j) {
        const int t = min(wave_m_u + 4 * j, ntile - 1);
        const int row = (int)(((unsigned)t * tpr_magic) >> 16);
        trow[j] = row;
        tcol0[j] = (t - row * tpr) * 16;
        base[j] = row * a.rs + tcol0[j];
    }
    const v4u rsx = make_srd(a.x, a.x_bytes);
    const v4u rsw = make_srd(a.w, a.w_bytes);
    constexpr unsigned OOB = 0x80000000u;
    const int wave_u = __builtin_amdgcn_readfirstlane(wave);
    const unsigned lds_base = (unsigned)(uintptr_t)(__attribute__((address_space(3))) char*)smem;
    const int patch_bytes = a.pra * 32;
    {
        const int npp = (a.pra + PPP - 1) / PPP;
        for (int piece = 0; piece < npp; ++piece) {
            if (piece * PPP + wave_u * 32 < a.pra) {
                const int t = piece * PPP + (tid >> 1);
                const int h = tid & 1;
                unsigned v[1] = {(unsigned)((p0 + t) * 32 + h * 16)};
                if (a.segs > 1) {
                    const int row = t / a.rs;
                    const int col = t - row * a.rs;
                    v[0] = cs0 + col < a.Ws ? (unsigned)((p0 + row * a.Ws + col) * 32 + h * 16) : OOB;
                }
                lds_dma16_group<1, 0>(rsx, v, 0u, lds_base + piece * (PPP * 32) + wave_u * 1024);
            }
        }
        const int ld_row = tid >> 3, ld_chunk = tid & 7;
        const int gch = ld_chunk ^ (ld_row & 7);
        const unsigned woff[1] = {ld_row < a.Cout ? (unsigned)(ld_row * a.w_row_bytes + gch * 16) : OOB};
        for (int kh = 0; kh < a.KH; ++kh)
            lds_dma16_group<1, 0>(rsw, woff, (unsigned)__builtin_amdgcn_readfirstlane(kh * 128), lds_base + patch_bytes + kh * (BN * 128) + wave_u * 1024);
    }
    asm volatile("s_waitcnt vmcnt(0)" ::: "memory");
    __syncthreads();

    const int rd_w = (wave_n * 32 + r16) * 128;
    uint2 res[NT][MT];
#pragma unroll
    for (int ps = 0; ps < NPASS; ++ps) {
        f32x4 acc[NT][MTP];
#pragma unroll
        for (int i = 0; i < NT; ++i)
#pragma unroll
            for (int jj = 0; jj < MTP; ++jj) acc[i][jj] = bias4v[i];
#pragma unroll 1
        for (int kh = 0; kh < a.KH; ++kh) {
            const char* wb = smem + patch_bytes + kh * (BN * 128);
#pragma unroll
            for (int kk = 0; kk < 2; ++kk) {
                const int sww = ((kk * 4 + q) ^ (r16 & 7)) << 4;
                uint4 fw[NT];
#pragma unroll
                for (int i = 0; i < NT; ++i) fw[i] = *(const uint4*)(wb + rd_w + i * 16 * 128 + sww);
#pragma unroll
                for (int j0 = 0; j0 < MTP; j0 += 5) {
                    uint4 fx[5];
#pragma unroll
                    for (int jj = j0; jj < MTP && jj < j0 + 5; ++jj) {
                        const int j = ps * MTP + jj < MT ? ps * MTP + jj : MT - 1;
                        const int pix = lane_px + (base[j] + kh * a.rs + kk * 2);
                        fx[jj - j0] = *(const uint4*)(smem + pix * 32 + ((q & 1) << 4));
                    }
                    asm volatile("" ::: "memory");
#pragma unroll
                    for (int i = 0; i < NT; ++i)
#pragma unroll
                        for (int jj = j0; jj < MTP && jj < j0 + 5; ++jj)
                            acc[i][jj] = __builtin_amdgcn_mfma_f32_16x16x32_bf16(__builtin_bit_cast(bf16x8_t, fw[i]), __builtin_bit_cast(bf16x8_t, fx[jj - j0]),
                                                                                 acc[i][jj], 0, 0, 0);
                }
            }
        }
#pragma unroll
        for (int i = 0; i < NT; ++i)
#pragma unroll
            for (int jj = 0; jj < MTP; ++jj)
                if (ps * MTP + jj < MT) {
                    uint2 o = make_uint2(pack_bf16x2(acc[i][jj][0], acc[i][jj][1]), pack_bf16x2(acc[i][jj][2], acc[i][jj][3]));
                    asm("v_pk_max_i16 %0, %0, 0" : "+v"(o.x));
                    asm("v_pk_max_i16 %0, %0, 0" : "+v"(o.y));
                    res[i][ps * MTP + jj] = o;
                }
    }
    __syncthreads();

    int wr_lane[NT];
#pragma unroll
    for (int i = 0; i < NT; ++i) {
        const int cb = (wave_n * 32 + i * 16 + q * 4) * 2;
        wr_lane[i] = r16 * 128 + (((cb >> 4) ^ ((r16 >> 1) & 7)) << 4) + (cb & 8);
    }
#pragma unroll
    for (int j = 0; j < MT; ++j) {
        if (wave_m_u + 4 * j < ntile) {
            const int col0 = tcol0[j];
            const int wr_tile = (trow[j] * a.ctw + col0) * 128;
            if (col0 + r16 < a.ctw) {
#pragma unroll
                for (int i = 0; i < NT; ++i) *(uint2*)(smem + wr_tile + wr_lane[i]) = res[i][j];
            }
        }
    }
    __syncthreads();

    const int nvec = 2 * a.wp_seg * 8;
    for (int v = tid; v < nvec; v += NTH) {
        const int c8 = v & 7;
        const int pp = v >> 3;
        const int pr = pp >= a.wp_seg ? 1 : 0;
        const int pc = Q0 + pp - pr * a.wp_seg;
        const int P = P0 + pr;
        if (P >= a.Hp || pc >= a.Wp || c8 * 8 >= a.Cout) continue;
        int roff[3], coff[3];
#pragma unroll
        for (int k = 0; k < 3; ++k) {
            const int jr = min(max(2 * pr + k, -c0), a.Ho - 1 - c0);
            roff[k] = jr * a.ctw * 128;
            const int cr = min(max(2 * pc - 1 + k, 0), a.Wo - 1) - cs0;
            coff[k] = cr * 128 + ((c8 ^ ((cr >> 1) & 7)) << 4);
        }
        uint4 best = make_uint4(0u, 0u, 0u, 0u);
#pragma unroll
        for (int kh = 0; kh < 3; ++kh)
#pragma unroll
            for (int kw = 0; kw < 3; ++kw) {
                const uint4 t = *(const uint4*)(smem + roff[kh] + coff[kw]);
                asm("v_pk_max_u16 %0, %0, %1" : "+v"(best.x) : "v"(t.x));
                asm("v_pk_max_u16 %0, %0, %1" : "+v"(best.y) : "v"(t.y));
                asm("v_pk_max_u16 %0, %0, %1" : "+v"(best.z) : "v"(t.z));
                asm("v_pk_max_u16 %0, %0, %1" : "+v"(best.w) : "v"(t.w));
            }
        *(uint4*)(a.y + (((long long)img * a.Hp + P) * a.Wp + pc) * (a.Cout * 2) + c8 * 16) = best;
    }
}

namespace {

struct TileCfg {
    int bm, bn;
};
constexpr TileCfg kTiles[] = {
    {128, 128}, {128, 64}, {64, 64}, {64, 128}, {32, 64}, {32, 32},
    {128, 128}, {64, 128}, {64, 64}, {32, 64}, {32, 32}, {128, 64},
    {256, 128}, {256, 128}, {256, 256}, {128, 256}, {256, 256}, {256, 128}, {256, 128}, {256, 64},
    {256, 64}, {256, 128}, {256, 256}, {256, 64}, {256, 128}, {256, 128},
    {256, 64}, {512, 64}, {128, 64}, {128, 128}, {256, 64}, {256, 128},
    {256, 64}, {256, 64},
    {32, 32}, {32, 64}, {32, 32}, {32, 32},
    {64, 64}, {64, 64}, {64, 64}, {64, 128}};
constexpr int kNumTiles = sizeof(kTiles) / sizeof(kTiles[0]);

template <typename T, int BM, int BN, int WM_, int WN_, int STAGES, bool OUT_F32, int KS = 1>
int launch_tile(const ConvK& k, bool fast, hipStream_t s) {
    const int m_tiles = cdiv(k.M, BM);
    ConvK kk = k;
    constexpr bool CAN_STATS = KS == 1 && WM_ * WN_ * BN * 16 <= (BM + BN) * 128;
    if (k.stat_sums && (!CAN_STATS || (k.Cout % (OUT_F32 ? 4 : 8)) != 0)) return MT4_EUNSUPPORTED;
    kk.n_tiles = cdiv(k.Cout, BN);
    kk.total_tiles = m_tiles * kk.n_tiles;
    kk.nt_epi = 1;
    {
        const long long min_mb = MT4_NT_MIN_MB;
        if ((long long)k.M * k.Cout * 2 < min_mb * 1000000LL) kk.nt_epi = 0;
    }
    constexpr int stage = (BM + BN) * 128;
    constexpr int os = OUT_F32 ? 4 : 2;
    constexpr int rowb = BN * 4 + 16;
    constexpr int passes = (BM * rowb > 4 * stage) ? 4 : (BM * rowb > 2 * stage) ? 2 : 1;
    constexpr int epi = BM / passes * rowb;
    constexpr int threads = WM_ * WN_ * 64;
    (void)os;
    if constexpr (KS > 1) {
        if (!fast) return MT4_EUNSUPPORTED;
        constexpr int lds_ks = KS * STAGES * stage > epi ? KS * STAGES * stage : epi;
        auto fn = igemm_conv_kernel<T, BM, BN, WM_, WN_, STAGES, true, OUT_F32, KS>;
        if (lds_ks > 65536) {
            MT4_RAISE_LDS(fn);
        }
        hipLaunchKernelGGL(fn, dim3(kk.total_tiles), dim3(threads * KS), lds_ks, s, kk);
        return mt4_check_launch();
    } else {
    const int lds = k.nsteps > 1 ? (fast ? STAGES : 2) * stage : (stage > epi ? stage : epi);
    const int grid = kk.total_tiles;
    if constexpr (CAN_STATS) {
        if (k.stat_sums) {
            if (fast) {
                auto fn = igemm_conv_kernel<T, BM, BN, WM_, WN_, STAGES, true, OUT_F32, 1, false, true>;
                if (lds > 65536) {
                    MT4_RAISE_LDS(fn);
                }
                hipLaunchKernelGGL(fn, dim3(grid), dim3(threads), lds, s, kk);
            } else {
                auto fn = igemm_conv_kernel<T, BM, BN, WM_, WN_, 2, false, OUT_F32, 1, false, true>;
                if (lds > 65536) {
                    MT4_RAISE_LDS(fn);
                }
                hipLaunchKernelGGL(fn, dim3(grid), dim3(threads), lds, s, kk);
            }
            return mt4_check_launch();
        }
    }
    if (fast) {
        auto fn = igemm_conv_kernel<T, BM, BN, WM_, WN_, STAGES, true, OUT_F32>;
        if (lds > 65536) {
            MT4_RAISE_LDS(fn);
        }
        hipLaunchKernelGGL(fn, dim3(grid), dim3(threads), lds, s, kk);
    } else {
        auto fn = igemm_conv_kernel<T, BM, BN, WM_, WN_, 2, false, OUT_F32>;
        if (lds > 65536) {
            MT4_RAISE_LDS(fn);
        }
        hipLaunchKernelGGL(fn, dim3(grid), dim3(threads), lds, s, kk);
    }
    return mt4_check_launch();
    }
}

int launch_dual(const ConvK& k, hipStream_t s) {
    constexpr int BM = 256, BN = 256, stage = (BM + BN) * 128;
    ConvK kk = k;
    kk.n_tiles = cdiv(k.Cout, BN);
    kk.total_tiles = cdiv(k.M, BM) * kk.n_tiles;
    kk.nt_epi = 1;
    if ((long long)k.M * k.Cout * 2 < (long long)MT4_NT_MIN_MB * 1000000LL) kk.nt_epi = 0;
    auto fn = igemm_conv_kernel<u16, BM, BN, 4, 4, 2, true, false, 1, true>;
    MT4_RAISE_LDS(fn);
    hipLaunchKernelGGL(fn, dim3(kk.total_tiles), dim3(1024), 2 * stage, s, kk);
    return mt4_check_launch();
}

template <typename T, bool OUT_F32>
int launch_dtype(const ConvK& k, int tile, bool fast, hipStream_t s) {
    switch (tile) {
        case 1: return launch_tile<T, 128, 128, 2, 2, 2, OUT_F32>(k, fast, s);
        case 2: return launch_tile<T, 128, 64, 2, 2, 2, OUT_F32>(k, fast, s);
        case 3: return launch_tile<T, 64, 64, 2, 2, 2, OUT_F32>(k, fast, s);
        case 4: return launch_tile<T, 64, 128, 2, 2, 2, OUT_F32>(k, fast, s);
        case 5: return launch_tile<T, 32, 64, 1, 4, 2, OUT_F32>(k, fast, s);
        case 6: return launch_tile<T, 32, 32, 2, 2, 2, OUT_F32>(k, fast, s);
        case 7: return launch_tile<T, 128, 128, 2, 2, 3, OUT_F32>(k, fast, s);
        case 8: return launch_tile<T, 64, 128, 2, 2, 3, OUT_F32>(k, fast, s);
        case 9: return launch_tile<T, 64, 64, 2, 2, 4, OUT_F32>(k, fast, s);
        case 10: return launch_tile<T, 32, 64, 1, 4, 4, OUT_F32>(k, fast, s);
        case 11: return launch_tile<T, 32, 32, 2, 2, 4, OUT_F32>(k, fast, s);
        case 12: return launch_tile<T, 128, 64, 2, 2, 3, OUT_F32>(k, fast, s);
        case 13: return launch_tile<T, 256, 128, 4, 2, 2, OUT_F32>(k, fast, s);
        case 14: return launch_tile<T, 256, 128, 4, 2, 3, OUT_F32>(k, fast, s);
        case 15: return launch_tile<T, 256, 256, 2, 4, 2, OUT_F32>(k, fast, s);
        case 16: return launch_tile<T, 128, 256, 2, 4, 3, OUT_F32>(k, fast, s);
        case 17: return launch_tile<T, 256, 256, 4, 4, 2, OUT_F32>(k, fast, s);
        case 18: return launch_tile<T, 256, 128, 4, 4, 2, OUT_F32>(k, fast, s);
        case 19: return launch_tile<T, 256, 128, 4, 4, 3, OUT_F32>(k, fast, s);
        case 20: return launch_tile<T, 256, 64, 4, 2, 2, OUT_F32>(k, fast, s);
        case 35: return launch_tile<T, 32, 32, 2, 2, 2, OUT_F32, 4>(k, fast, s);
        case 36: return launch_tile<T, 32, 64, 1, 4, 2, OUT_F32, 4>(k, fast, s);
        case 37: return launch_tile<T, 32, 32, 1, 2, 2, OUT_F32, 8>(k, fast, s);
        case 38: return launch_tile<T, 32, 32, 2, 2, 3, OUT_F32, 4>(k, fast, s);
        case 39: return launch_tile<T, 64, 64, 2, 2, 2, OUT_F32, 2>(k, fast, s);
        case 40: return launch_tile<T, 64, 64, 2, 2, 2, OUT_F32, 4>(k, fast, s);
        case 41: return launch_tile<T, 64, 64, 2, 2, 3, OUT_F32, 2>(k, fast, s);
        case 42: return launch_tile<T, 64, 128, 2, 2, 2, OUT_F32, 2>(k, fast, s);
    }
    return MT4_EINVAL;
}


bool patch3x3_ok(const mt4_conv_desc* d, const ConvK& k, bool fast) {
    return fast && d->dtype == MT4_BF16 && d->out_dtype == MT4_BF16 && d->KH == 3 && d->KW == 3 && d->stride_h == 1 && d->stride_w == 1 &&
           d->dil_h == 1 && d->dil_w == 1 && d->pad_h == 1 && d->pad_w == 1 && d->Ho == d->H && d->Wo == d->W && k.pix_bytes == d->Cin * 2 &&
           !d->out_row_map && d->relu <= 1 && (d->Cout % 8) == 0 && k.nsteps == 9 * k.SPT && (!d->residual || (k.res_ld * 2) % 16 == 0) &&
           k.x_total_bytes + (long long)(2 * d->W + 1024) * k.pix_bytes < 0x7fffffffLL;
}

template <int BM, int BN, int WM_, int WN_, int WS, bool EXPAND = false>
int launch_patch3x3(const ConvK& k, hipStream_t s) {
    ConvK kk = k;
    kk.n_tiles = cdiv(k.Cout, BN);
    kk.total_tiles = cdiv(k.M, BM) * kk.n_tiles;
    kk.nt_epi = 1;
    {
        const long long min_mb = MT4_NT_MIN_MB;
        if ((long long)k.M * (EXPAND ? k.f_cout : k.Cout) * 2 < min_mb * 1000000LL) kk.nt_epi = 0;
    }
    constexpr int threads = WM_ * WN_ * 64;
    constexpr int rpp = threads / 8;
    const int pra = (BM + 2 * k.W + 2 + 2 + 7) / 8 * 8;
    const int npatch = k.SPT > 1 ? 2 : 1;
    constexpr int epi = BM / (BN >= 256 ? 4 : 2) * (BN * 4 + 16);
    int lds = npatch * pra * 128 + WS * BN * 128;
    if (lds < epi) lds = epi;
    if (EXPAND && lds < 2 * BM * 128 + epi) lds = 2 * BM * 128 + epi;
    if (WS == 9 && k.SPT != 1) return MT4_EUNSUPPORTED;
    if (lds > 160 * 1024 || (k.SPT > 1 && cdiv(pra, rpp) > 11 - WS)) return MT4_EUNSUPPORTED;
    if (k.stat_sums && (EXPAND || (k.Cout & 7))) return MT4_EUNSUPPORTED;
    if constexpr (!EXPAND) {
        if (k.stat_sums) {
            auto fs = conv3x3_patch_kernel<BM, BN, WM_, WN_, WS, false, true>;
            if (lds > 65536) {
                MT4_RAISE_LDS(fs);
            }
            hipLaunchKernelGGL(fs, dim3(kk.total_tiles), dim3(threads), lds, s, kk, pra, npatch);
            return mt4_check_launch();
        }
    }
    auto fn = conv3x3_patch_kernel<BM, BN, WM_, WN_, WS, EXPAND, false>;
    if (lds > 65536) {
        MT4_RAISE_LDS(fn);
    }
    hipLaunchKernelGGL(fn, dim3(kk.total_tiles), dim3(threads), lds, s, kk, pra, npatch);
    return mt4_check_launch();
}

int launch_patch_tile(const ConvK& k, int tile, hipStream_t s) {
    switch (tile) {
        case 23: return launch_patch3x3<256, 256, 4, 4, 2>(k, s);
        case 24: return launch_patch3x3<256, 64, 4, 2, 2>(k, s);
        case 26: return launch_patch3x3<256, 128, 4, 4, 2>(k, s);
        case 30: return launch_patch3x3<128, 128, 2, 2, 2>(k, s);
        case 32: return launch_patch3x3<256, 128, 4, 2, 2>(k, s);
    }
    return MT4_EUNSUPPORTED;
}

bool stem_patch_ok(const mt4_conv_desc* d, const ConvK& k, bool fast) {
    return fast && d->dtype == MT4_BF16 && d->out_dtype == MT4_BF16 && d->KW == 1 && d->KH <= 8 && d->Cin == 64 && k.pix_bytes == 32 &&
           d->stride_h == 1 && d->stride_w == 1 && d->dil_h == 1 && d->dil_w == 1 && d->pad_h == 0 && d->pad_w == 0 &&
           d->W == d->Wo + 3 && d->H == d->Ho + d->KH - 1 && !d->residual && !d->out_row_map && d->relu <= 1 && d->Cout <= 64 &&
           (d->Cout % 8) == 0 && k.HoWo >= 256 && k.nsteps == d->KH && k.x_total_bytes < 0x70000000LL;
}

int launch_stem_patch(const ConvK& k, hipStream_t s) {
    constexpr int BM = 256;
    ConvK kk = k;
    kk.n_tiles = 1;
    kk.total_tiles = cdiv(k.M, BM);
    kk.nt_epi = 1;
    {
        const long long min_mb = MT4_NT_MIN_MB;
        if ((long long)k.M * k.Cout * 2 < min_mb * 1000000LL) kk.nt_epi = 0;
    }
    kk.n_tiles = cdiv(k.HoWo, BM);
    kk.total_tiles = k.B * kk.n_tiles;
    const int rows_crossed = cdiv(BM, k.Wo) + 1;
    const int span = BM + 3 * rows_crossed + (k.KH - 1) * k.W + 4;
    const int pra = (span + 31) / 32 * 32;
    int lds = pra * 32 + k.KH * 64 * 128;
    constexpr int epi = BM / 2 * (64 * 4 + 16);
    if (lds < epi) lds = epi;
    if (lds > 160 * 1024) return MT4_EUNSUPPORTED;
    auto fn = stem_patch_kernel<BM, 4, 2>;
    if (lds > 65536) {
        MT4_RAISE_LDS(fn);
    }
    hipLaunchKernelGGL(fn, dim3(kk.total_tiles), dim3(512), lds, s, kk, pra);
    return mt4_check_launch();
}

int auto_tile(int M, int N, int nsteps, int es) {
    auto tiles = [&](int t) { return (long long)cdiv(M, kTiles[t - 1].bm) * cdiv(N, kTiles[t - 1].bn); };
    const long long fill = 256;
    if (es == 2 && N >= 256) {
        if (nsteps == 1 && tiles(13) >= fill) return 13;
        if (nsteps >= 2 && tiles(15) >= 190) return 17;
    }
    if (es == 2 && N > 64 && N <= 128 && nsteps < 4 && tiles(20) >= 8 * fill) {
        return 20;
    }
    if (es == 2 && N > 64 && N <= 128 && nsteps >= 4 && tiles(19) >= 8 * fill) {
        return 19;
    }
    if (nsteps == 1 && tiles(3) >= 4 * fill) return 3;
    if (N > 64) {
        if (nsteps >= 4 && tiles(1) >= fill) return 1;
        if (tiles(4) >= fill) return 4;
        if (tiles(1) >= fill) return 1;
    } else if (N > 32) {
        if (es == 2 && tiles(20) >= 8 * fill) return 20;
        if (tiles(2) >= fill) return 2;
        if (tiles(3) >= fill) return 3;
    }
    if (nsteps >= 32 && N > 32 && tiles(3) >= 192) return 9;
    int best = 6;
    long long best_tiles = -1;
    for (int t = 1; t <= 6; ++t) {
        if (kTiles[t - 1].bn > 64 && N <= 64) continue;
        if (kTiles[t - 1].bn > 32 && N <= 32) continue;
        if (tiles(t) > best_tiles) {
            best_tiles = tiles(t);
            best = t;
        }
    }
    if (nsteps >= 8) {
        if (best == 5) return 10;
        if (best == 6) return 11;
        if (best == 3) return 9;
    }
    return best;
}

}

extern "C" int mt4_conv_tile_count(void) { return kNumTiles; }

extern "C" int64_t mt4_conv_packed_k(int32_t Cin, int32_t KH, int32_t KW, int32_t dtype) {
    const int es = dtype == MT4_BF16 ? 2 : 4;
    const int cpt = cdiv(Cin * es, 16);
    const int chunks = cdiv(KH * KW * cpt, 8) * 8;
    return (int64_t)chunks * (16 / es);
}

extern "C" int mt4_conv_nhwc(const mt4_conv_desc* d, void* stream) {
    mt4_clear_error();
    if (!d || !d->x || !d->w || !d->y) return MT4_EINVAL;
    if (d->B <= 0 || d->H <= 0 || d->W <= 0 || d->Cin <= 0 || d->Ho <= 0 || d->Wo <= 0 || d->Cout <= 0 || d->KH <= 0 ||
        d->KW <= 0 || d->stride_h <= 0 || d->stride_w <= 0 || d->dil_h <= 0 || d->dil_w <= 0)
        return MT4_EINVAL;
    if (d->dtype != MT4_F32 && d->dtype != MT4_BF16) return MT4_EUNSUPPORTED;
    if (d->out_dtype != MT4_F32 && d->out_dtype != MT4_BF16) return MT4_EUNSUPPORTED;
    if (d->dtype == MT4_F32 && d->out_dtype != MT4_F32) return MT4_EUNSUPPORTED;
    const int es = d->dtype == MT4_BF16 ? 2 : 4;
    if ((d->Cin * es) % 16 != 0) return MT4_EALIGN;
    if (((uintptr_t)d->x | (uintptr_t)d->w | (uintptr_t)d->y | (uintptr_t)d->residual | (uintptr_t)d->bias) & 15) return MT4_EALIGN;
    const long long M = (long long)d->B * d->Ho * d->Wo;
    if (M > 0x7fffffffLL || M * d->Cout * 4 > (1LL << 40)) return MT4_EUNSUPPORTED;

    ConvK k{};
    k.x = (const char*)d->x; k.w = (const char*)d->w; k.bias = d->bias; k.res = (const char*)d->residual; k.y = (char*)d->y;
    k.B = d->B; k.H = d->H; k.W = d->W; k.Cin = d->Cin; k.Ho = d->Ho; k.Wo = d->Wo; k.Cout = d->Cout;
    k.KH = d->KH; k.KW = d->KW; k.sh = d->stride_h; k.sw = d->stride_w; k.ph = d->pad_h; k.pw = d->pad_w;
    k.dh = d->dil_h; k.dw = d->dil_w; k.relu = d->relu;
    if (d->relu < 0 || d->relu > 3) return MT4_EINVAL;
    if (d->relu == 3 && !d->residual) return MT4_EINVAL;
    k.row_map = d->out_row_map; k.map_len = d->out_row_map_len;
    k.map_img = d->out_rows_per_image > 0 ? d->out_rows_per_image : d->out_row_map_len;
    k.y_ld = d->y_ld > 0 ? d->y_ld : d->Cout;
    k.res_ld = d->res_ld > 0 ? d->res_ld : d->Cout;
    if (k.y_ld < d->Cout || k.res_ld < d->Cout) return MT4_EINVAL;
    if (d->residual_float && !(d->dtype == MT4_BF16 && d->out_dtype == MT4_F32 && !d->fuse_w)) return MT4_EUNSUPPORTED;
    k.res_f32 = d->residual_float ? 1 : 0;
    {
        const int oes = d->out_dtype == MT4_BF16 ? 2 : 4;
        const int res_es = k.res_f32 ? 4 : es;
        if ((d->Cout * oes) % 16 == 0 && ((k.y_ld * oes) % 16 != 0 || (d->residual && (k.res_ld * res_es) % 16 != 0))) return MT4_EALIGN;
    }
    if (d->out_row_map && d->out_row_map_len <= 0) return MT4_EINVAL;
    k.M = (int)M; k.HoWo = d->Ho * d->Wo;
    if (d->KH == 1 && d->KW == 1 && d->stride_h == 1 && d->stride_w == 1 && d->pad_h == 0 && d->pad_w == 0) {
        k.B = (int)M; k.H = k.W = k.Ho = k.Wo = 1; k.HoWo = 1;
    }
    k.CPT = (d->Cin * es) / 16;
    k.taps = d->KH * d->KW;
    k.nsteps = cdiv(k.taps * k.CPT, 8);
    k.w_row_bytes = k.nsteps * 128;
    const int pix = (d->x_pixel_stride > 0 ? d->x_pixel_stride : d->Cin) * es;
    if (pix % 16 != 0 || pix > d->Cin * es) return MT4_EALIGN;
    if (pix != d->Cin * es && (d->KW != 1 || d->pad_w != 0 || d->pad_h != 0)) return MT4_EUNSUPPORTED;
    k.pix_bytes = pix;
    k.x_img_bytes = (long long)k.H * k.W * pix;
    const long long xb = (long long)d->B * d->H * d->W * pix, wb = (long long)d->Cout * k.w_row_bytes;
    const long long tile_span = ((long long)(256 / k.HoWo) + 2) * k.x_img_bytes +
                                ((long long)(d->KH - 1) * d->dil_h * d->W + (long long)(d->KW - 1) * d->dil_w) * pix + (long long)k.CPT * 16 + 4096;
    const bool fast = (k.CPT % 8) == 0 && tile_span + (((long long)d->pad_h * d->W + d->pad_w) * pix) < 0x70000000LL && wb < 0x7fffffffLL &&
                      d->KH <= 8 && d->KW <= 8;
    k.x_total_bytes = xb;
    k.x_bias = (unsigned)(((long long)d->pad_h * d->W + d->pad_w) * pix);
    k.x_bytes = (unsigned)(xb < 0x7fffffffLL ? xb : 0);
    k.w_bytes = (unsigned)(wb < 0x7fffffffLL ? wb : 0);
    k.SPT = fast ? k.CPT / 8 : 1;
    if (d->stat_sums) {
        if ((uintptr_t)d->stat_sums & 7) return MT4_EALIGN;
        if (d->fuse_w || d->x2 || d->out_row_map || d->tile == -1 || d->tile == 33 || pix != d->Cin * es) return MT4_EUNSUPPORTED;
        k.stat_sums = d->stat_sums;
    }
    if (d->fuse_w && d->fuse_expand) {
        if (!d->fuse_y || !d->fuse_bias || d->fuse_cout <= 0 || (d->fuse_cout % 128) != 0) return MT4_EINVAL;
        if (((uintptr_t)d->fuse_w | (uintptr_t)d->fuse_y | (uintptr_t)d->fuse_bias) & 15) return MT4_EALIGN;
        if (!(patch3x3_ok(d, k, fast) && d->Cin == 128 && d->Cout == 128 && d->tile == 0 && !d->x2 &&
              (long long)cdiv(k.M, 256) * cdiv(d->fuse_cout, 256) >= 256))
            return MT4_EUNSUPPORTED;
        k.f_w = (const char*)d->fuse_w; k.f_bias = d->fuse_bias; k.f_y = (char*)d->fuse_y; k.f_cout = d->fuse_cout; k.f_relu = d->fuse_relu ? 1 : 0;
        return d->W <= 31 ? launch_patch3x3<128, 128, 2, 2, 2, true>(k, (hipStream_t)stream) : launch_patch3x3<256, 128, 4, 2, 2, true>(k, (hipStream_t)stream);
    }
    if (d->fuse_w) return MT4_EUNSUPPORTED;
    if (d->x2) {
        if (d->x2_H <= 0 || d->x2_W <= 0 || d->x2_C <= 0 || d->x2_stride <= 0) return MT4_EINVAL;
        if (!(fast && d->dtype == MT4_BF16 && d->out_dtype == MT4_BF16 && d->KH == 1 && d->KW == 1 && d->stride_h == 1 && d->stride_w == 1 &&
              d->pad_h == 0 && d->pad_w == 0 && !d->out_row_map && !d->residual && d->relu <= 1 && d->tile == 0 && pix == d->Cin * es &&
              (d->x2_C * 2) % 128 == 0 && (d->Cout % 8) == 0 && (k.y_ld * 2) % 16 == 0))
            return MT4_EUNSUPPORTED;
        if ((long long)(d->Ho - 1) * d->x2_stride >= d->x2_H || (long long)(d->Wo - 1) * d->x2_stride >= d->x2_W) return MT4_EINVAL;
        if ((uintptr_t)d->x2 & 15) return MT4_EALIGN;
        k.x2 = (const char*)d->x2;
        k.x2_pix_bytes = d->x2_C * 2;
        k.x2_img_bytes = (long long)d->x2_H * d->x2_W * k.x2_pix_bytes;
        k.x2_total_bytes = (long long)d->B * k.x2_img_bytes;
        k.x2_W = d->x2_W; k.x2_s = d->x2_stride; k.x2_HoWo = d->Ho * d->Wo; k.x2_Wo = d->Wo;
        if (((long long)(256 / k.x2_HoWo) + 2) * k.x2_img_bytes >= 0x70000000LL) return MT4_EUNSUPPORTED;
        k.nsteps1 = k.nsteps;
        k.nsteps += d->x2_C * 2 / 128;
        k.w_row_bytes = k.nsteps * 128;
        const long long wb2 = (long long)d->Cout * k.w_row_bytes;
        if (wb2 >= 0x7fffffffLL) return MT4_EUNSUPPORTED;
        k.w_bytes = (unsigned)wb2;
        return launch_dual(k, (hipStream_t)stream);
    }
    int tile = d->tile;
    if (tile < -1 || tile > kNumTiles) return MT4_EINVAL;
    const bool latency = tile == -1;
    if (latency) tile = 0;
    hipStream_t s = (hipStream_t)stream;
    if (tile == 34) return MT4_EUNSUPPORTED;
    if (tile == 33 || (tile == 0 && stem_patch_ok(d, k, fast))) {
        if (!stem_patch_ok(d, k, fast)) return MT4_EUNSUPPORTED;
        const int rc = launch_stem_patch(k, s);
        if (rc != MT4_EUNSUPPORTED || tile != 0) return rc;
    }
    if (tile >= 21 && tile <= 32) {
        if (!patch3x3_ok(d, k, fast)) return MT4_EUNSUPPORTED;
        return launch_patch_tile(k, tile, s);
    }
    if (tile == 0 && patch3x3_ok(d, k, fast) && (long long)cdiv(k.M, 256) * cdiv(k.Cout, 256) >= 256) {
        const int pt = d->Cout <= 64 ? 24 : d->Cout <= 128 ? (d->W <= 31 ? 30 : 32) : 23;
        const int rc = launch_patch_tile(k, pt, s);
        if (rc != MT4_EUNSUPPORTED) return rc;
    }
    if (tile == 0) {
        tile = auto_tile(k.M, k.Cout, k.nsteps, d->dtype == MT4_F32 ? 4 : 2);
        if (latency && fast && d->dtype == MT4_F32 && (tile == 10 || tile == 11)) {
            const int kt = tile == 11 ? 37 : 36;
            if ((long long)cdiv(k.M, kTiles[kt - 1].bm) * cdiv(k.Cout, kTiles[kt - 1].bn) <= 256) tile = kt;
        }
        if (latency && tile == 1) {
            const long long t128 = (long long)cdiv(k.M, 128) * cdiv(k.Cout, 128), t64 = (long long)cdiv(k.M, 64) * cdiv(k.Cout, 128);
            if (t128 < 512 && t64 >= 256) tile = 4;
        }
        if (latency && fast && k.nsteps >= 8 && (tile == 5 || tile == 6 || tile == 10 || tile == 11 || tile == 3 || tile == 9)) {
            const long long t64 = (long long)cdiv(k.M, 64) * cdiv(k.Cout, 64);
            if (t64 >= 192 && t64 <= 512) tile = d->dtype == MT4_F32 ? 40 : 41;
            else if (d->dtype == MT4_BF16 && tile == 11 && (long long)cdiv(k.M, 32) * cdiv(k.Cout, 64) >= 256) tile = 10;
        }
    }
    if (d->dtype == MT4_F32) return launch_dtype<float, true>(k, tile, fast, s);
    if (d->out_dtype == MT4_F32) return launch_dtype<u16, true>(k, tile, fast, s);
    return launch_dtype<u16, false>(k, tile, fast, s);
}

template <typename T>
__global__ void pack_conv_weight_kernel(const float* __restrict__ w, const float* __restrict__ scale, T* __restrict__ out,
                                        int Cout, int Cin, int KH, int KW, int CPT_E, long long Kpad) {
    const long long idx = (long long)blockIdx.x * blockDim.x + threadIdx.x;
    if (idx >= (long long)Cout * Kpad) return;
    const int n = (int)(idx / Kpad);
    const long long k = idx - (long long)n * Kpad;
    const int tap = (int)(k / CPT_E);
    const int c = (int)(k - (long long)tap * CPT_E);
    float v = 0.f;
    if (tap < KH * KW && c < Cin) {
        const int kh = tap / KW, kw = tap - kh * KW;
        v = w[(((long long)n * Cin + c) * KH + kh) * KW + kw];
        if (scale) v *= scale[n];
    }
    if constexpr (sizeof(T) == 2) out[idx] = f32_to_bf16(v);
    else out[idx] = v;
}

extern "C" int mt4_pack_conv_weight(const float* w_oihw, const float* scale, void* w_packed, int32_t Cout, int32_t Cin,
                                    int32_t KH, int32_t KW, int32_t dtype, void* stream) {
    mt4_clear_error();
    if (!w_oihw || !w_packed || Cout <= 0 || Cin <= 0 || KH <= 0 || KW <= 0) return MT4_EINVAL;
    if (dtype != MT4_F32 && dtype != MT4_BF16) return MT4_EUNSUPPORTED;
    const int es = dtype == MT4_BF16 ? 2 : 4;
    const int E = 16 / es;
    const int cpt = cdiv(Cin * es, 16);
    const long long Kpad = mt4_conv_packed_k(Cin, KH, KW, dtype);
    const long long total = (long long)Cout * Kpad;
    const int grid = (int)((total + 255) / 256);
    hipStream_t s = (hipStream_t)stream;
    if (dtype == MT4_BF16)
        hipLaunchKernelGGL(pack_conv_weight_kernel<u16>, dim3(grid), dim3(256), 0, s, w_oihw, scale, (u16*)w_packed, Cout, Cin,
                           KH, KW, cpt * E, Kpad);
    else
        hipLaunchKernelGGL(pack_conv_weight_kernel<float>, dim3(grid), dim3(256), 0, s, w_oihw, scale, (float*)w_packed, Cout,
                           Cin, KH, KW, cpt * E, Kpad);
    return mt4_check_launch();
}

extern "C" int mt4_stem_maxpool_bf16(const void* x_s2d, const void* w_packed, const float* bias, void* y, int32_t B, int32_t Hs, int32_t Ws,
                                     int32_t Cout, int32_t KH, void* stream) {
    mt4_clear_error();
    if (!x_s2d || !w_packed || !y || B <= 0 || Hs <= 0 || Ws <= 3 || KH <= 0 || KH > Hs) return MT4_EINVAL;
    if (((uintptr_t)x_s2d | (uintptr_t)w_packed | (uintptr_t)y | (uintptr_t)bias) & 15) return MT4_EALIGN;
    const int Ho = Hs - KH + 1, Wo = Ws - 3;
    if (KH > 8 || Cout != 64 || (Wo & 15) || Wo > 224) return MT4_EUNSUPPORTED;
    const long long xb = (long long)B * Hs * Ws * 32;
    if (xb >= 0x70000000LL) return MT4_EUNSUPPORTED;
    StemPoolK k{};
    k.x = (const char*)x_s2d; k.w = (const char*)w_packed; k.bias = bias; k.y = (char*)y;
    k.x_bytes = (unsigned)xb;
    k.w_row_bytes = KH * 128;
    k.w_bytes = (unsigned)(Cout * k.w_row_bytes);
    k.Cout = Cout; k.KH = KH; k.Hs = Hs; k.Ws = Ws; k.Ho = Ho; k.Wo = Wo;
    k.Hp = (Ho - 1) / 2 + 1; k.Wp = (Wo - 1) / 2 + 1;
    const bool wide = Wo > 112;
    k.segs = wide ? 2 : 1;
    k.cw = wide ? 128 : Wo;
    k.rs = wide ? 132 : Ws;
    k.wp_seg = wide ? cdiv(k.Wp, 2) : k.Wp;
    k.ctw = k.cw < 2 * k.wp_seg + 8 ? k.cw : 2 * k.wp_seg + 8;
    k.tiles_per_img = cdiv(k.Hp, 2) * k.segs;
    k.pra = ((4 + KH) * k.rs + 31) / 32 * 32;
    int lds = k.pra * 32 + KH * 64 * 128;
    if (lds < 5 * k.ctw * 128) lds = 5 * k.ctw * 128;
    if (lds > 80 * 1024) return MT4_EUNSUPPORTED;
    if ((long long)B * k.tiles_per_img > 0x7fffffffLL) return MT4_EUNSUPPORTED;
    if (wide) {
        auto fn = stem_pool_kernel<10, 2>;
        MT4_RAISE_LDS(fn);
        hipLaunchKernelGGL(fn, dim3((unsigned)(B * k.tiles_per_img)), dim3(512), lds, (hipStream_t)stream, k);
    } else {
        auto fn = stem_pool_kernel<9, 2>;
        if (lds > 65536) MT4_RAISE_LDS(fn);
        hipLaunchKernelGGL(fn, dim3((unsigned)(B * k.tiles_per_img)), dim3(512), lds, (hipStream_t)stream, k);
    }
    return mt4_check_launch();
}

template <typename T>
__global__ void pack_stem_weight_kernel(const float* __restrict__ w, const float* __restrict__ scale, T* __restrict__ out,
                                        int Cout, long long Kpad) {
    const long long idx = (long long)blockIdx.x * blockDim.x + threadIdx.x;
    if (idx >= (long long)Cout * Kpad) return;
    const int n = (int)(idx / Kpad);
    const int k = (int)(idx - (long long)n * Kpad);
    const int tap = k >> 3, slot = k & 7;
    const int kh = tap >> 2, kwp = tap & 3;
    const int kw = 2 * kwp + (slot >> 2), c = slot & 3;
    float v = 0.f;
    if (kh < 7 && kw < 7 && c < 3) {
        v = w[(((long long)n * 3 + c) * 7 + kh) * 7 + kw];
        if (scale) v *= scale[n];
    }
    if constexpr (sizeof(T) == 2) out[idx] = f32_to_bf16(v);
    else out[idx] = v;
}

extern "C" int mt4_pack_stem_weight(const float* w_oihw, const float* scale, void* w_packed, int32_t Cout, int32_t dtype,
                                    void* stream) {
    mt4_clear_error();
    if (!w_oihw || !w_packed || Cout <= 0) return MT4_EINVAL;
    if (dtype != MT4_F32 && dtype != MT4_BF16) return MT4_EUNSUPPORTED;
    const long long Kpad = mt4_conv_packed_k(8, 7, 4, dtype);
    const long long total = (long long)Cout * Kpad;
    const int grid = (int)((total + 255) / 256);
    hipStream_t s = (hipStream_t)stream;
    if (dtype == MT4_BF16)
        hipLaunchKernelGGL(pack_stem_weight_kernel<u16>, dim3(grid), dim3(256), 0, s, w_oihw, scale, (u16*)w_packed, Cout, Kpad);
    else
        hipLaunchKernelGGL(pack_stem_weight_kernel<float>, dim3(grid), dim3(256), 0, s, w_oihw, scale, (float*)w_packed, Cout,
                           Kpad);
    return mt4_check_launch();
}
```

computervision_codes_amd/csrc/mt4_common.h:

```cpp
#pragma once
#include <hip/hip_runtime.h>
#include <stdint.h>
#include <stdlib.h>

#include "../../include/mt4hip.h"

typedef float f32x4 __attribute__((ext_vector_type(4)));
typedef short bf16x8 __attribute__((ext_vector_type(8)));
typedef unsigned short u16;

extern thread_local int g_mt4_last_hip_error;

static inline void mt4_clear_error() { (void)hipGetLastError(); }

static inline int mt4_check_launch() {
    hipError_t e = hipGetLastError();
    if (e != hipSuccess) {
        g_mt4_last_hip_error = (int)e;
        return MT4_ELAUNCH;
    }
    return MT4_OK;
}

__device__ __forceinline__ float bf16_to_f32(u16 v) { return __uint_as_float(((uint32_t)v) << 16); }

typedef __bf16 bf16x2_t __attribute__((ext_vector_type(2)));
typedef float f32x2_t __attribute__((ext_vector_type(2)));

__device__ __forceinline__ u16 f32_to_bf16(float f) {
    const __bf16 b = (__bf16)f;
    return __builtin_bit_cast(u16, b);
}

__device__ __forceinline__ uint32_t pack_bf16x2(float lo, float hi) {
    const f32x2_t v = {lo, hi};
    return __builtin_bit_cast(uint32_t, __builtin_convertvector(v, bf16x2_t));
}

typedef float mt4_f32x2 __attribute__((ext_vector_type(2)));
__device__ __forceinline__ mt4_f32x2 gelu_erf2(mt4_f32x2 x) {
    const mt4_f32x2 a = {fminf(fabsf(x.x), 6.0f), fminf(fabsf(x.y), 6.0f)};
    mt4_f32x2 p = a * 4.881283152809e-04f + -7.198873334067e-03f;
    p = p * a + 5.214694370026e-02f;
    p = p * a + 4.595955966962e-01f;
    p = p * a + 1.151000605814e+00f;
    const mt4_f32x2 q = p * a;
    const mt4_f32x2 t = {__builtin_amdgcn_exp2f(-q.x), __builtin_amdgcn_exp2f(-q.y)};
    const mt4_f32x2 u = 1.0f - t;
    const mt4_f32x2 hx = x * 0.5f;
    const mt4_f32x2 s = {__builtin_copysignf(u.x, x.x), __builtin_copysignf(u.y, x.y)};
    return hx * s + hx;
}
__device__ __forceinline__ float gelu_erf(float x) {
    const float a = fminf(fabsf(x), 6.0f);
    float p = fmaf(a, 4.881283152809e-04f, -7.198873334067e-03f);
    p = fmaf(p, a, 5.214694370026e-02f);
    p = fmaf(p, a, 4.595955966962e-01f);
    p = fmaf(p, a, 1.151000605814e+00f);
    const float t = __builtin_amdgcn_exp2f(-(p * a));
    const float hx = 0.5f * x;
    return fmaf(hx, __builtin_copysignf(1.0f - t, x), hx);
}
template <int N>
__device__ __forceinline__ void gelu_erf_n(float (&v)[N]) {
    static_assert(N % 2 == 0, "pairs");
#pragma unroll
    for (int e = 0; e < N; e += 2) {
        const mt4_f32x2 r = gelu_erf2((mt4_f32x2){v[e], v[e + 1]});
        v[e] = r.x; v[e + 1] = r.y;
    }
}

static inline int cdiv(int a, int b) { return (a + b - 1) / b; }

#define MT4_RAISE_LDS(fn)                                                                                                   \
    do {                                                                                                                    \
        static bool raised_[64] = {};                                                                                       \
        int dev_ = 0;                                                                                                       \
        (void)hipGetDevice(&dev_);                                                                                          \
        if (dev_ < 0 || dev_ >= 64 || !raised_[dev_]) {                                                                     \
            (void)hipFuncSetAttribute((const void*)(fn), hipFuncAttributeMaxDynamicSharedMemorySize, 160 * 1024);           \
            if (dev_ >= 0 && dev_ < 64) raised_[dev_] = true;                                                               \
        }                                                                                                                   \
    } while (0)

#define MT4_NT_MIN_MB 200
```

Before: 97070.

## Make fused bottleneck kernel persistent with LDS-DMA prefetch of next tile

Converts the fused ResNet bottleneck kernel from one-workgroup-per-tile to a persistent grid sized to twice the CU count, where each workgroup walks a contiguous run of tiles in column-major tile order. Input halo chunks are now loaded with buffer_load...lds direct-to-LDS DMA instead of going through registers, and the next tile's chunks are issued during the current tile's 3x3 conv and output stages, so global loads overlap compute. Biases are cached in LDS once, w1 fragments are reused across tiles, and the identity block stages output in t2/t1 so xs is free for prefetch. This adds LDS footprint, extra barriers and vmcnt waits, and more register pressure in exchange for hiding load latency and launch/tail overhead.

```diff
diff --git a/computervision_codes_amd/csrc/bottleneck_fused.hip b/computervision_codes_amd/csrc/bottleneck_fused.hip
--- a/computervision_codes_amd/csrc/bottleneck_fused.hip
+++ b/computervision_codes_amd/csrc/bottleneck_fused.hip
@@ -10,6 +10,16 @@
 constexpr int T2_BYTES = NPX * ROW_B;
 constexpr int T1_BYTES = XS_BYTES + 2 * ROW_B;
 constexpr int YS_BYTES = NPX * 256;
+constexpr int DMA_PASS = 4 * 8 * ROW_B;
+constexpr unsigned DMA_OOB = 0x80000000u;
+
+template <int CIN, bool DS, bool NEXT>
+struct BneckLds {
+    static constexpr int NXS = CIN > 64 ? 2 : 1;
+    static constexpr int BIAS = NXS * XS_BYTES + T2_BYTES + (DS ? YS_BYTES : T1_BYTES);
+    static constexpr int NBIAS = 64 + 64 + 256 + (DS ? 256 : 0) + (NEXT ? 128 : 0);
+    static constexpr int BYTES = BIAS + NBIAS * 4;
+};
 
 struct BneckK {
     const char* x;
@@ -17,6 +27,7 @@
     const char *w1, *w2, *w3, *wds;
     const float *b1, *b2, *b3, *bds;
     int B, H, W, tiles_h, tiles_w;
+    int ntiles;
     int nt;
     char* y2;
     const char* wn;
@@ -40,327 +51,409 @@
     return __builtin_amdgcn_mfma_f32_16x16x32_bf16(__builtin_bit_cast(bf16x8_t, wfrag), __builtin_bit_cast(bf16x8_t, xfrag), acc, 0, 0, 0);
 }
 
+template <int N>
+__device__ __forceinline__ void vm_wait() {
+    static_assert(N >= 0 && N < 16, "vmcnt");
+    __builtin_amdgcn_s_waitcnt((0xF << 8) | (0x7 << 4) | N);
+    asm volatile("" ::: "memory");
+}
+
 template <int CIN, bool DS, bool NEXT = false>
 __global__ __launch_bounds__(256, 2) void bottleneck64_fused_kernel(const BneckK a) {
     static_assert(!NEXT || !DS, "the following conv rides behind an identity block");
     constexpr int KC = CIN / 64;
-    constexpr int NXS = KC > 1 ? 2 : 1;
     static_assert(DS ? CIN == 64 : CIN == 256, "layer1.0 (64 channels in, downsample branch) or layer1.1+ (256 in, identity)");
+    using L = BneckLds<CIN, DS, NEXT>;
+    constexpr int NXS = L::NXS;
     extern __shared__ __attribute__((aligned(16))) char smem[];
     char* const xs = smem;
     char* const t2 = smem + NXS * XS_BYTES;
     char* const t1 = t2 + T2_BYTES;
-    char* const ys = DS ? t1 : xs;
+    char* const ys = DS ? t1 : t2;
+    float* const bs = (float*)(smem + L::BIAS);
 
     const int tid = threadIdx.x;
-    const int lane = tid & 63, wave = tid >> 6;
-    const int r16 = lane & 15, q = lane >> 4;
-
-    int bid = blockIdx.x;
+    const unsigned wave_u = __builtin_amdgcn_readfirstlane(tid >> 6);
+    const unsigned lds_base = (unsigned)(uintptr_t)(__attribute__((address_space(3))) char*)smem;
+    auto chunk_buf = [&](int kc) -> char* { return kc == 2 ? t1 : xs + (kc == 1 ? XS_BYTES : 0); };
+
+    {
+        for (int i = tid; i < L::NBIAS; i += 256) {
+            float v;
+            if (i < 64) v = a.b1[i];
+            else if (i < 128) v = a.b2[i - 64];
+            else if (i < 384) v = a.b3[i - 128];
+            else v = DS ? a.bds[i - 384] : a.bn[i - 384];
+            bs[i] = v;
+        }
+    }
+
+    int run0, run1;
     {
         const int nb = gridDim.x;
         const int q8 = nb >> 3, r8 = nb & 7;
-        const int xcd = bid & 7, local = bid >> 3;
-        bid = (xcd < r8 ? xcd * (q8 + 1) : r8 * (q8 + 1) + (xcd - r8) * q8) + local;
+        const int xcd = blockIdx.x & 7, local = blockIdx.x >> 3;
+        const int lb = (xcd < r8 ? xcd * (q8 + 1) : r8 * (q8 + 1) + (xcd - r8) * q8) + local;
+        run0 = (int)((long long)lb * a.ntiles / nb);
+        run1 = (int)((long long)(lb + 1) * a.ntiles / nb);
     }
     const int tpi = a.tiles_h * a.tiles_w;
-    const int img = bid / tpi;
-    const int trem = bid - img * tpi;
-    const int th = trem / a.tiles_w;
-    const int h0 = th * TH, w0 = (trem - th * a.tiles_w) * TW;
-    const char* const ximg = a.x + (long long)img * a.H * a.W * (CIN * 2);
-    char* const yimg = NEXT ? a.y + (long long)img * a.H2 * a.W2 * 512 : a.y + (long long)img * a.H * a.W * 512;
-
-    const int ld_row = tid >> 3, ld_chunk = tid & 7;
-    int xoff[5];
-#pragma unroll
-    for (int i = 0; i < 5; ++i) {
-        const int hp = ld_row + 32 * i;
-        const int h = h0 - 1 + (hp >> 4), w = w0 - 1 + (hp & 15);
-        xoff[i] = ((unsigned)h < (unsigned)a.H && (unsigned)w < (unsigned)a.W) ? (h * a.W + w) * (CIN * 2) + ld_chunk * 16 : -1;
-    }
-    auto load_chunk = [&](int kc, uint4 (&stg)[5]) {
+    auto tile_of = [&](int t, int& img, int& h0, int& w0) {
+        img = t / tpi;
+        const int r = t - img * tpi;
+        const int col = r / a.tiles_h;
+        h0 = (r - col * a.tiles_h) * TH;
+        w0 = col * TW;
+    };
+
+    auto issue_chunk = [&](int kc, int img, int h0, int w0) {
+        int tid_d = tid;
+        asm volatile("" : "+v"(tid_d));
+        const int lr = (tid_d >> 3) & 7, gch = (tid_d & 7) ^ lr, hp0 = 8 * (tid_d >> 6) + lr;
+        const v4u srd = make_srd(a.x + (long long)img * a.H * a.W * (CIN * 2), (unsigned)(a.H * a.W * (CIN * 2)));
+        unsigned voff4[4], voff1[1];
 #pragma unroll
         for (int i = 0; i < 5; ++i) {
-            stg[i] = make_uint4(0, 0, 0, 0);
-            if (xoff[i] >= 0) stg[i] = *(const uint4*)(ximg + xoff[i] + kc * 128);
-        }
+            const int hp = 32 * i + hp0;
+            const int h = h0 - 1 + (hp >> 4), w = w0 - 1 + (hp & 15);
+            const unsigned o = ((unsigned)h < (unsigned)a.H && (unsigned)w < (unsigned)a.W) ? (unsigned)((h * a.W + w) * (CIN * 2) + gch * 16) : DMA_OOB;
+            if (i < 4) voff4[i] = o; else voff1[0] = o;
+        }
+        const unsigned dst = lds_base + (unsigned)(chunk_buf(kc) - smem) + wave_u * 1024;
+        lds_dma16_group<4, DMA_PASS>(srd, voff4, (unsigned)(kc * 128), dst);
+        lds_dma16_group<1, 0>(srd, voff1, (unsigned)(kc * 128), dst + 4 * DMA_PASS);
     };
-    auto store_chunk = [&](int buf, const uint4 (&stg)[5]) {
-#pragma unroll
-        for (int i = 0; i < 5; ++i) {
-            const int hp = ld_row + 32 * i;
-            *(uint4*)(xs + buf * XS_BYTES + hp * ROW_B + ((ld_chunk ^ (hp & 7)) << 4)) = stg[i];
-        }
+
+    int img, h0, w0;
+    tile_of(run0, img, h0, w0);
+    issue_chunk(0, img, h0, w0);
+    if constexpr (KC > 1) issue_chunk(1, img, h0, w0);
+
+    uint4 wf1[KC * 2];
+    auto load_wf1 = [&]() {
+        int tid_w = tid;
+        asm volatile("" : "+v"(tid_w));
+        const char* wr = a.w1 + (((tid_w >> 6) * (KC * 2) * 64 + (tid_w & 63)) * 16);
+#pragma unroll
+        for (int s = 0; s < KC * 2; ++s) wf1[s] = *(const uint4*)(wr + s * 1024);
     };
-    uint4 stg0[5], stg1[5];
-    load_chunk(0, stg0);
-    if constexpr (KC > 1) load_chunk(1, stg1);
-
-    const int ch1 = wave * 16;
-    uint4 wf1[KC * 2];
-    {
-        const char* wr = a.w1 + (wave * (KC * 2) * 64 + lane) * 16;
-#pragma unroll
-        for (int s = 0; s < KC * 2; ++s) wf1[s] = *(const uint4*)(wr + s * 1024);
-    }
-    f32x4 acc1[10];
-    {
-        const f32x4 b4 = bias4(a.b1, ch1 + q * 4);
-#pragma unroll
-        for (int i = 0; i < 10; ++i) acc1[i] = b4;
-    }
-    const int sw0 = (q ^ (r16 & 7)) << 4, sw1 = ((4 + q) ^ (r16 & 7)) << 4;
-    uint2 res[DS ? 1 : 4][DS ? 1 : 8];
-    const int res_off = (r16 + 1) * ROW_B + (((2 * wave + (q >> 1)) ^ ((r16 + 1) & 7)) << 4) + (q & 1) * 8;
-#pragma unroll
-    for (int kc = 0; kc < KC; ++kc) {
-        if (kc & 1) store_chunk(1, stg1); else store_chunk(0, stg0);
-        if (kc + 2 < KC) { if (kc & 1) load_chunk(kc + 2, stg1); else load_chunk(kc + 2, stg0); }
+    load_wf1();
+    __syncthreads();
+
+#pragma unroll 1
+    for (int t = run0; t < run1; ++t) {
+        const bool more = t + 1 < run1;
+        int tid_t = tid;
+        asm volatile("" : "+v"(tid_t));
+        const int lane = tid_t & 63, wave = tid_t >> 6;
+        const int r16 = lane & 15, q = lane >> 4;
+        const int ch1 = wave * 16;
+        const int sw0 = (q ^ (r16 & 7)) << 4, sw1 = ((4 + q) ^ (r16 & 7)) << 4;
+        const int res_off = (r16 + 1) * ROW_B + (((2 * wave + (q >> 1)) ^ ((r16 + 1) & 7)) << 4) + (q & 1) * 8;
+        const int cb1 = (ch1 + q * 4) * 2;
+        int toff[3][2];
+#pragma unroll
+        for (int kw = 0; kw < 3; ++kw)
+#pragma unroll
+            for (int kk = 0; kk < 2; ++kk) toff[kw][kk] = (r16 + kw) * ROW_B + (((kk * 4 + q) ^ ((r16 + kw) & 7)) << 4);
+        const int st_tx = tid >> 4, st_chunk = tid & 15;
+
+        int nimg, nh0, nw0;
+        tile_of(t + 1, nimg, nh0, nw0);
+        char* const yimg = NEXT ? a.y + (long long)img * a.H2 * a.W2 * 512 : a.y + (long long)img * a.H * a.W * 512;
+
+        f32x4 acc1[10];
+        {
+            const f32x4 b4 = bias4(bs, ch1 + q * 4);
+#pragma unroll
+            for (int i = 0; i < 10; ++i) acc1[i] = b4;
+        }
+        uint2 res[DS ? 1 : 4][DS ? 1 : 8];
+#pragma unroll
+        for (int kc = 0; kc < KC; ++kc) {
+            if (kc == 0 || kc == KC - 1) vm_wait<0>();
+            else vm_wait<5>();
+            __syncthreads();
+            if (kc + 2 < KC) issue_chunk(kc + 2, img, h0, w0);
+            const char* sb = chunk_buf(kc) + r16 * ROW_B;
+            uint4 fx[2][10];
+#pragma unroll
+            for (int kk = 0; kk < 2; ++kk)
+#pragma unroll
+                for (int i = 0; i < 10; ++i) fx[kk][i] = *(const uint4*)(sb + i * 16 * ROW_B + (kk ? sw1 : sw0));
+            if constexpr (!DS) {
+#pragma unroll
+                for (int j = 0; j < 8; ++j) res[kc][j] = *(const uint2*)(chunk_buf(kc) + (j + 1) * (16 * ROW_B) + res_off);
+            }
+            asm volatile("" ::: "memory");
+#pragma unroll
+            for (int kk = 0; kk < 2; ++kk)
+#pragma unroll
+                for (int i = 0; i < 10; ++i) acc1[i] = mfma_bf16(wf1[kc * 2 + kk], fx[kk][i], acc1[i]);
+        }
+        uint4 wf2[18];
+        {
+            const char* wr = a.w2 + (wave * 18 * 64 + lane) * 16;
+#pragma unroll
+            for (int s = 0; s < 18; ++s) wf2[s] = *(const uint4*)(wr + s * 1024);
+        }
+        {
+            const int wr_off = r16 * ROW_B + (((cb1 >> 4) ^ (r16 & 7)) << 4) + (cb1 & 8);
+            const int w = w0 - 1 + r16;
+#pragma unroll
+            for (int i = 0; i < 10; ++i) {
+                const int h = h0 - 1 + i;
+                const bool in = (unsigned)h < (unsigned)a.H && (unsigned)w < (unsigned)a.W;
+                uint2 o = make_uint2(0, 0);
+                if (in) o = relu_pack4(acc1[i]);
+                *(uint2*)(t1 + i * (16 * ROW_B) + wr_off) = o;
+            }
+        }
         __syncthreads();
-        const char* sb = xs + (kc & 1) * XS_BYTES + r16 * ROW_B;
-        uint4 fx[2][10];
-#pragma unroll
-        for (int kk = 0; kk < 2; ++kk)
-#pragma unroll
-            for (int i = 0; i < 10; ++i) fx[kk][i] = *(const uint4*)(sb + i * 16 * ROW_B + (kk ? sw1 : sw0));
-        if constexpr (!DS) {
-#pragma unroll
-            for (int j = 0; j < 8; ++j) res[kc][j] = *(const uint2*)(xs + (kc & 1) * XS_BYTES + (j + 1) * (16 * ROW_B) + res_off);
-        }
-        asm volatile("" ::: "memory");
-#pragma unroll
-        for (int kk = 0; kk < 2; ++kk)
-#pragma unroll
-            for (int i = 0; i < 10; ++i) acc1[i] = mfma_bf16(wf1[kc * 2 + kk], fx[kk][i], acc1[i]);
-    }
-    uint4 wf2[18];
-    {
-        const char* wr = a.w2 + (wave * 18 * 64 + lane) * 16;
-#pragma unroll
-        for (int s = 0; s < 18; ++s) wf2[s] = *(const uint4*)(wr + s * 1024);
-    }
-    const int cb1 = (ch1 + q * 4) * 2;
-    {
-        const int wr_off = r16 * ROW_B + (((cb1 >> 4) ^ (r16 & 7)) << 4) + (cb1 & 8);
-        const int w = w0 - 1 + r16;
-#pragma unroll
-        for (int i = 0; i < 10; ++i) {
-            const int h = h0 - 1 + i;
-            const bool in = (unsigned)h < (unsigned)a.H && (unsigned)w < (unsigned)a.W;
-            uint2 o = make_uint2(0, 0);
-            if (in) o = relu_pack4(acc1[i]);
-            *(uint2*)(t1 + i * (16 * ROW_B) + wr_off) = o;
-        }
-    }
-    __syncthreads();
-
-    f32x4 acc2[8];
-    {
-        const f32x4 b4 = bias4(a.b2, ch1 + q * 4);
-#pragma unroll
-        for (int j = 0; j < 8; ++j) acc2[j] = b4;
-    }
-    int toff[3][2];
-#pragma unroll
-    for (int kw = 0; kw < 3; ++kw)
-#pragma unroll
-        for (int kk = 0; kk < 2; ++kk) toff[kw][kk] = (r16 + kw) * ROW_B + (((kk * 4 + q) ^ ((r16 + kw) & 7)) << 4);
-#pragma unroll
-    for (int hr = 0; hr < 10; ++hr) {
-        uint4 fr[3][2];
-#pragma unroll
-        for (int kw = 0; kw < 3; ++kw)
-#pragma unroll
-            for (int kk = 0; kk < 2; ++kk) fr[kw][kk] = *(const uint4*)(t1 + hr * (16 * ROW_B) + toff[kw][kk]);
-        asm volatile("" ::: "memory");
-#pragma unroll
-        for (int kh = 0; kh < 3; ++kh) {
-            const int ty = hr - kh;
-            if (ty >= 0 && ty < 8) {
-#pragma unroll
-                for (int kw = 0; kw < 3; ++kw)
-#pragma unroll
-                    for (int kk = 0; kk < 2; ++kk) acc2[ty] = mfma_bf16(wf2[(kh * 3 + kw) * 2 + kk], fr[kw][kk], acc2[ty]);
-            }
-        }
-    }
-    uint4 wf3[4][2];
-    uint4 wfd[DS ? 4 : 1][2];
-#pragma unroll
-    for (int i = 0; i < 4; ++i) {
-        const char* wr = a.w3 + ((4 * i + wave) * 2 * 64 + lane) * 16;
-        wf3[i][0] = *(const uint4*)wr;
-        wf3[i][1] = *(const uint4*)(wr + 1024);
-        if constexpr (DS) {
-            const char* wd = a.wds + ((4 * i + wave) * 2 * 64 + lane) * 16;
-            wfd[i][0] = *(const uint4*)wd;
-            wfd[i][1] = *(const uint4*)(wd + 1024);
-        }
-    }
-    {
-        const int wr_off = r16 * ROW_B + (((cb1 >> 4) ^ (r16 & 7)) << 4) + (cb1 & 8);
+
+        f32x4 acc2[8];
+        {
+            const f32x4 b4 = bias4(bs + 64, ch1 + q * 4);
+#pragma unroll
+            for (int j = 0; j < 8; ++j) acc2[j] = b4;
+        }
+#pragma unroll
+        for (int hr = 0; hr < 10; ++hr) {
+            uint4 fr[3][2];
+#pragma unroll
+            for (int kw = 0; kw < 3; ++kw)
+#pragma unroll
+                for (int kk = 0; kk < 2; ++kk) fr[kw][kk] = *(const uint4*)(t1 + hr * (16 * ROW_B) + toff[kw][kk]);
+            asm volatile("" ::: "memory");
+#pragma unroll
+            for (int kh = 0; kh < 3; ++kh) {
+                const int ty = hr - kh;
+                if (ty >= 0 && ty < 8) {
+#pragma unroll
+                    for (int kw = 0; kw < 3; ++kw)
+#pragma unroll
+                        for (int kk = 0; kk < 2; ++kk) acc2[ty] = mfma_bf16(wf2[(kh * 3 + kw) * 2 + kk], fr[kw][kk], acc2[ty]);
+                }
+            }
+            if constexpr (!DS && !NEXT) {
+                if (hr == 2 && more) {
+                    vm_wait<0>();
+                    issue_chunk(0, nimg, nh0, nw0);
+                }
+            }
+        }
+        uint4 wf3[4][2];
+        uint4 wfd[DS ? 4 : 1][2];
+#pragma unroll
+        for (int i = 0; i < 4; ++i) {
+            const char* wr = a.w3 + ((4 * i + wave) * 2 * 64 + lane) * 16;
+            wf3[i][0] = *(const uint4*)wr;
+            wf3[i][1] = *(const uint4*)(wr + 1024);
+            if constexpr (DS) {
+                const char* wd = a.wds + ((4 * i + wave) * 2 * 64 + lane) * 16;
+                wfd[i][0] = *(const uint4*)wd;
+                wfd[i][1] = *(const uint4*)(wd + 1024);
+            }
+        }
+        {
+            const int wr_off = r16 * ROW_B + (((cb1 >> 4) ^ (r16 & 7)) << 4) + (cb1 & 8);
+#pragma unroll
+            for (int j = 0; j < 8; ++j) {
+                const uint2 o = relu_pack4(acc2[j]);
+                *(uint2*)(t2 + j * (16 * ROW_B) + wr_off) = o;
+            }
+        }
+        __syncthreads();
+
+        uint4 fx3[8][2];
 #pragma unroll
         for (int j = 0; j < 8; ++j) {
-            const uint2 o = relu_pack4(acc2[j]);
-            *(uint2*)(t2 + j * (16 * ROW_B) + wr_off) = o;
-        }
-    }
-    __syncthreads();
-
-    uint4 fx3[8][2];
-#pragma unroll
-    for (int j = 0; j < 8; ++j) {
-        fx3[j][0] = *(const uint4*)(t2 + j * (16 * ROW_B) + r16 * ROW_B + sw0);
-        fx3[j][1] = *(const uint4*)(t2 + j * (16 * ROW_B) + r16 * ROW_B + sw1);
-    }
-    const int st_tx = tid >> 4, st_chunk = tid & 15;
-    uint4 wfn[NEXT ? 2 : 1][NEXT ? 8 : 1];
-#pragma unroll
-    for (int pass = 0; pass < 2; ++pass) {
-        char* const ysp = NEXT ? xs + pass * YS_BYTES : ys;
-        if (pass && !NEXT) __syncthreads();
-#pragma unroll
-        for (int ii = 0; ii < 2; ++ii) {
-            const int i = pass * 2 + ii;
-            const int ct = 4 * i + wave;
-            f32x4 acc3[8];
+            fx3[j][0] = *(const uint4*)(t2 + j * (16 * ROW_B) + r16 * ROW_B + sw0);
+            fx3[j][1] = *(const uint4*)(t2 + j * (16 * ROW_B) + r16 * ROW_B + sw1);
+        }
+        if constexpr (!DS && !NEXT) {
+            __syncthreads();
+            vm_wait<0>();
+            if (more) issue_chunk(1, nimg, nh0, nw0);
+        }
+        uint4 wfn[NEXT ? 2 : 1][NEXT ? 8 : 1];
+#pragma unroll
+        for (int pass = 0; pass < 2; ++pass) {
+            char* const ysp = NEXT ? xs + pass * YS_BYTES : ys;
+            if (pass && !NEXT) __syncthreads();
+            if constexpr (!DS && !NEXT) {
+                if (pass == 1) load_wf1();
+            }
+#pragma unroll
+            for (int ii = 0; ii < 2; ++ii) {
+                const int i = pass * 2 + ii;
+                const int ct = 4 * i + wave;
+                f32x4 acc3[8];
+                {
+                    const f32x4 b4 = bias4(bs + 128, ct * 16 + q * 4);
+#pragma unroll
+                    for (int j = 0; j < 8; ++j) acc3[j] = b4;
+                }
+#pragma unroll
+                for (int kk = 0; kk < 2; ++kk)
+#pragma unroll
+                    for (int j = 0; j < 8; ++j) acc3[j] = mfma_bf16(wf3[i][kk], fx3[j][kk], acc3[j]);
+                if constexpr (DS) {
+                    const f32x4 bd4 = bias4(bs + 384, ct * 16 + q * 4);
+#pragma unroll
+                    for (int j = 0; j < 8; ++j) {
+                        f32x4 accd = bd4;
+#pragma unroll
+                        for (int kk = 0; kk < 2; ++kk) accd = mfma_bf16(wfd[i][kk], *(const uint4*)(xs + (j + 1) * (16 * ROW_B) + toff[1][kk]), accd);
+#pragma unroll
+                        for (int e = 0; e < 4; ++e) acc3[j][e] += bf16_to_f32(f32_to_bf16(accd[e]));
+                    }
+                } else {
+#pragma unroll
+                    for (int j = 0; j < 8; ++j) {
+                        acc3[j][0] += __uint_as_float(res[i][j].x << 16);
+                        acc3[j][1] += __uint_as_float(res[i][j].x & 0xffff0000u);
+                        acc3[j][2] += __uint_as_float(res[i][j].y << 16);
+                        acc3[j][3] += __uint_as_float(res[i][j].y & 0xffff0000u);
+                    }
+                }
+                const int cbyte = ((ct - 8 * pass) * 16 + q * 4) * 2;
+                const int wr_off = r16 * 256 + (((cbyte >> 4) ^ r16) << 4) + (cbyte & 8);
+#pragma unroll
+                for (int j = 0; j < 8; ++j) {
+                    const uint2 o = relu_pack4(acc3[j]);
+                    *(uint2*)(ysp + j * (16 * 256) + wr_off) = o;
+                }
+            }
+            if constexpr (NEXT) {
+                if (pass == 1) {
+#pragma unroll
+                    for (int c = 0; c < 2; ++c)
+#pragma unroll
+                        for (int ks = 0; ks < 8; ++ks) wfn[c][ks] = *(const uint4*)(a.wn + (((2 * wave + c) * 8 + ks) * 64 + lane) * 16);
+                }
+            }
+            __syncthreads();
+            if constexpr (DS) {
+                if (pass == 1) {
+                    if (more) issue_chunk(0, nimg, nh0, nw0);
+                    load_wf1();
+                }
+            }
             {
-                const f32x4 b4 = bias4(a.b3, ct * 16 + q * 4);
-#pragma unroll
-                for (int j = 0; j < 8; ++j) acc3[j] = b4;
-            }
-#pragma unroll
-            for (int kk = 0; kk < 2; ++kk)
-#pragma unroll
-                for (int j = 0; j < 8; ++j) acc3[j] = mfma_bf16(wf3[i][kk], fx3[j][kk], acc3[j]);
-            if constexpr (DS) {
-                const f32x4 bd4 = bias4(a.bds, ct * 16 + q * 4);
-#pragma unroll
-                for (int j = 0; j < 8; ++j) {
-                    f32x4 accd = bd4;
-#pragma unroll
-                    for (int kk = 0; kk < 2; ++kk) accd = mfma_bf16(wfd[i][kk], *(const uint4*)(xs + (j + 1) * (16 * ROW_B) + toff[1][kk]), accd);
-#pragma unroll
-                    for (int e = 0; e < 4; ++e) acc3[j][e] += bf16_to_f32(f32_to_bf16(accd[e]));
-                }
-            } else {
-#pragma unroll
-                for (int j = 0; j < 8; ++j) {
-                    acc3[j][0] += __uint_as_float(res[i][j].x << 16);
-                    acc3[j][1] += __uint_as_float(res[i][j].x & 0xffff0000u);
-                    acc3[j][2] += __uint_as_float(res[i][j].y << 16);
-                    acc3[j][3] += __uint_as_float(res[i][j].y & 0xffff0000u);
-                }
-            }
-            const int cbyte = ((ct - 8 * pass) * 16 + q * 4) * 2;
-            const int wr_off = r16 * 256 + (((cbyte >> 4) ^ r16) << 4) + (cbyte & 8);
-#pragma unroll
-            for (int j = 0; j < 8; ++j) {
-                const uint2 o = relu_pack4(acc3[j]);
-                *(uint2*)(ysp + j * (16 * 256) + wr_off) = o;
+                const int w = w0 + st_tx;
+                const int rd_off = st_tx * 256 + ((st_chunk ^ st_tx) << 4);
+                if constexpr (NEXT) {
+                    if (st_tx < TW && w < a.W && !(st_tx & 1)) {
+                        const uint4 v0 = *(const uint4*)(ysp + rd_off), v1 = *(const uint4*)(ysp + 2 * (16 * 256) + rd_off);
+                        const uint4 v2 = *(const uint4*)(ysp + 4 * (16 * 256) + rd_off), v3 = *(const uint4*)(ysp + 6 * (16 * 256) + rd_off);
+                        char* const yp = yimg + (unsigned)(((h0 >> 1) * a.W2 + (w >> 1)) * 512 + pass * 256 + st_chunk * 16);
+                        const int rows = a.H - h0;
+                        *(uint4*)yp = v0;
+                        if (rows > 2) *(uint4*)(yp + a.W2 * 512) = v1;
+                        if (rows > 4) *(uint4*)(yp + 2 * a.W2 * 512) = v2;
+                        if (rows > 6) *(uint4*)(yp + 3 * a.W2 * 512) = v3;
+                    }
+                } else if (st_tx < TW && w < a.W) {
+                    uint4 v[8];
+#pragma unroll
+                    for (int ty = 0; ty < 8; ++ty) v[ty] = *(const uint4*)(ysp + ty * (16 * 256) + rd_off);
+                    asm volatile("" ::: "memory");
+#pragma unroll
+                    for (int ty = 0; ty < 8; ++ty) {
+                        if (h0 + ty < a.H) {
+                            typedef unsigned u32x4 __attribute__((ext_vector_type(4)));
+                            char* yp = yimg + (unsigned)((h0 + ty) * a.W * 512) + (unsigned)(w * 512 + pass * 256 + st_chunk * 16);
+                            if (a.nt) __builtin_nontemporal_store((u32x4){v[ty].x, v[ty].y, v[ty].z, v[ty].w}, (u32x4*)yp);
+                            else *(uint4*)yp = v[ty];
+                        }
+                    }
+                }
             }
         }
         if constexpr (NEXT) {
-            if (pass == 1) {
+            f32x4 acc4[2][8];
+#pragma unroll
+            for (int c = 0; c < 2; ++c) {
+                const f32x4 b4 = bias4(bs + 384, (2 * wave + c) * 16 + q * 4);
+#pragma unroll
+                for (int j = 0; j < 8; ++j) acc4[c][j] = b4;
+            }
+#pragma unroll
+            for (int ks = 0; ks < 8; ++ks) {
+                uint4 fy[8];
+                const char* yb = xs + (ks >> 2) * YS_BYTES + r16 * 256 + ((((ks & 3) * 4 + q) ^ r16) << 4);
+#pragma unroll
+                for (int j = 0; j < 8; ++j) fy[j] = *(const uint4*)(yb + j * (16 * 256));
+                asm volatile("" ::: "memory");
 #pragma unroll
                 for (int c = 0; c < 2; ++c)
 #pragma unroll
-                    for (int ks = 0; ks < 8; ++ks) wfn[c][ks] = *(const uint4*)(a.wn + (((2 * wave + c) * 8 + ks) * 64 + lane) * 16);
-            }
-        }
-        __syncthreads();
-        {
+                    for (int j = 0; j < 8; ++j) acc4[c][j] = mfma_bf16(wfn[c][ks], fy[j], acc4[c][j]);
+            }
+            __syncthreads();
+            if (more) {
+                issue_chunk(0, nimg, nh0, nw0);
+                issue_chunk(1, nimg, nh0, nw0);
+            }
+            load_wf1();
+            char* const y2s = t2;
+#pragma unroll
+            for (int c = 0; c < 2; ++c) {
+                const int cbyte = ((2 * wave + c) * 16 + q * 4) * 2;
+                const int wr_off = r16 * 256 + (((cbyte >> 4) ^ r16) << 4) + (cbyte & 8);
+#pragma unroll
+                for (int j = 0; j < 8; ++j) *(uint2*)(y2s + j * (16 * 256) + wr_off) = relu_pack4(acc4[c][j]);
+            }
+            __syncthreads();
             const int w = w0 + st_tx;
-            const int rd_off = st_tx * 256 + ((st_chunk ^ st_tx) << 4);
-            if constexpr (NEXT) {
-                if (st_tx < TW && w < a.W && !(st_tx & 1)) {
-                    const uint4 v0 = *(const uint4*)(ysp + rd_off), v1 = *(const uint4*)(ysp + 2 * (16 * 256) + rd_off);
-                    const uint4 v2 = *(const uint4*)(ysp + 4 * (16 * 256) + rd_off), v3 = *(const uint4*)(ysp + 6 * (16 * 256) + rd_off);
-                    char* const yp = yimg + (unsigned)(((h0 >> 1) * a.W2 + (w >> 1)) * 512 + pass * 256 + st_chunk * 16);
-                    const int rows = a.H - h0;
-                    *(uint4*)yp = v0;
-                    if (rows > 2) *(uint4*)(yp + a.W2 * 512) = v1;
-                    if (rows > 4) *(uint4*)(yp + 2 * a.W2 * 512) = v2;
-                    if (rows > 6) *(uint4*)(yp + 3 * a.W2 * 512) = v3;
-                }
-            } else if (st_tx < TW && w < a.W) {
+            if (st_tx < TW && w < a.W) {
+                const int rd_off = st_tx * 256 + ((st_chunk ^ st_tx) << 4);
+                char* const y2img = a.y2 + (long long)img * a.H * a.W * 256;
                 uint4 v[8];
 #pragma unroll
-                for (int ty = 0; ty < 8; ++ty) v[ty] = *(const uint4*)(ysp + ty * (16 * 256) + rd_off);
+                for (int ty = 0; ty < 8; ++ty) v[ty] = *(const uint4*)(y2s + ty * (16 * 256) + rd_off);
                 asm volatile("" ::: "memory");
 #pragma unroll
                 for (int ty = 0; ty < 8; ++ty) {
                     if (h0 + ty < a.H) {
                         typedef unsigned u32x4 __attribute__((ext_vector_type(4)));
-                        char* yp = yimg + (unsigned)((h0 + ty) * a.W * 512) + (unsigned)(w * 512 + pass * 256 + st_chunk * 16);
+                        char* yp = y2img + (unsigned)(((h0 + ty) * a.W + w) * 256 + st_chunk * 16);
                         if (a.nt) __builtin_nontemporal_store((u32x4){v[ty].x, v[ty].y, v[ty].z, v[ty].w}, (u32x4*)yp);
                         else *(uint4*)yp = v[ty];
                     }
                 }
             }
         }
+        img = nimg; h0 = nh0; w0 = nw0;
     }
-    if constexpr (NEXT) {
-        f32x4 acc4[2][8];
-#pragma unroll
-        for (int c = 0; c < 2; ++c) {
-            const f32x4 b4 = bias4(a.bn, (2 * wave + c) * 16 + q * 4);
-#pragma unroll
-            for (int j = 0; j < 8; ++j) acc4[c][j] = b4;
-        }
-#pragma unroll
-        for (int ks = 0; ks < 8; ++ks) {
-            uint4 fy[8];
-            const char* yb = xs + (ks >> 2) * YS_BYTES + r16 * 256 + ((((ks & 3) * 4 + q) ^ r16) << 4);
-#pragma unroll
-            for (int j = 0; j < 8; ++j) fy[j] = *(const uint4*)(yb + j * (16 * 256));
-            asm volatile("" ::: "memory");
-#pragma unroll
-            for (int c = 0; c < 2; ++c)
-#pragma unroll
-                for (int j = 0; j < 8; ++j) acc4[c][j] = mfma_bf16(wfn[c][ks], fy[j], acc4[c][j]);
-        }
-        __syncthreads();
-#pragma unroll
-        for (int c = 0; c < 2; ++c) {
-            const int cbyte = ((2 * wave + c) * 16 + q * 4) * 2;
-            const int wr_off = r16 * 256 + (((cbyte >> 4) ^ r16) << 4) + (cbyte & 8);
-#pragma unroll
-            for (int j = 0; j < 8; ++j) *(uint2*)(xs + j * (16 * 256) + wr_off) = relu_pack4(acc4[c][j]);
-        }
-        __syncthreads();
-        const int w = w0 + st_tx;
-        if (st_tx < TW && w < a.W) {
-            const int rd_off = st_tx * 256 + ((st_chunk ^ st_tx) << 4);
-            char* const y2img = a.y2 + (long long)img * a.H * a.W * 256;
-            uint4 v[8];
-#pragma unroll
-            for (int ty = 0; ty < 8; ++ty) v[ty] = *(const uint4*)(xs + ty * (16 * 256) + rd_off);
-            asm volatile("" ::: "memory");
-#pragma unroll
-            for (int ty = 0; ty < 8; ++ty) {
-                if (h0 + ty < a.H) {
-                    typedef unsigned u32x4 __attribute__((ext_vector_type(4)));
-                    char* yp = y2img + (unsigned)(((h0 + ty) * a.W + w) * 256 + st_chunk * 16);
-                    if (a.nt) __builtin_nontemporal_store((u32x4){v[ty].x, v[ty].y, v[ty].z, v[ty].w}, (u32x4*)yp);
-                    else *(uint4*)yp = v[ty];
-                }
-            }
-        }
+}
+
+static int bneck_slots() {
+    static int cus[64] = {};
+    int dev = 0;
+    (void)hipGetDevice(&dev);
+    if (dev >= 0 && dev < 64 && cus[dev]) return 2 * cus[dev];
+    int n = 0;
+    if (hipDeviceGetAttribute(&n, hipDeviceAttributeMultiprocessorCount, dev) != hipSuccess || n <= 0) {
+        (void)hipGetLastError();
+        n = 256;
     }
+    if (dev >= 0 && dev < 64) cus[dev] = n;
+    return 2 * n;
 }
 
 template <int CIN, bool DS, bool NEXT = false>
 int launch(const BneckK& a, hipStream_t stream) {
-    constexpr int NXS = CIN > 64 ? 2 : 1;
-    constexpr int LDS = NXS * XS_BYTES + T2_BYTES + (DS ? YS_BYTES : T1_BYTES);
+    constexpr int LDS = BneckLds<CIN, DS, NEXT>::BYTES;
     static_assert(LDS <= 80 * 1024, "two workgroups per CU");
-    static_assert(!NEXT || LDS >= 2 * YS_BYTES, "both output passes stay in LDS");
+    static_assert(!NEXT || BneckLds<CIN, DS, NEXT>::BIAS >= 2 * YS_BYTES, "both output passes stay in LDS");
+    static_assert(DS || T2_BYTES + T1_BYTES >= YS_BYTES, "identity blocks stage a pass in t2 | t1");
     auto fn = bottleneck64_fused_kernel<CIN, DS, NEXT>;
     MT4_RAISE_LDS(fn);
-    const long long nblk = (long long)a.B * a.tiles_h * a.tiles_w;
-    hipLaunchKernelGGL(fn, dim3((unsigned)nblk), dim3(256), LDS, stream, a);
+    const int slots = bneck_slots();
+    const unsigned grid = (unsigned)(a.ntiles < slots ? a.ntiles : slots);
+    hipLaunchKernelGGL(fn, dim3(grid), dim3(256), LDS, stream, a);
     return mt4_check_launch();
 }
 
@@ -410,7 +503,7 @@
     if (mid != 64 || !((ds && Cin == 64) || (!ds && Cin == 256))) return MT4_EUNSUPPORTED;
     if (((uintptr_t)x | (uintptr_t)y | (uintptr_t)w_frag | (uintptr_t)b1 | (uintptr_t)b2 | (uintptr_t)b3 | (uintptr_t)bds) & 15) return MT4_EALIGN;
     if ((long long)H * W * 512 > 0x7fffffffLL) return MT4_EUNSUPPORTED;
-    BneckK a;
+    BneckK a{};
     a.x = (const char*)x; a.y = (char*)y;
     const int k1 = Cin / 32;
     a.w1 = (const char*)w_frag;
@@ -422,6 +515,7 @@
     a.tiles_h = cdiv(H, TH); a.tiles_w = cdiv(W, TW);
     a.nt = 1;
     if ((long long)B * a.tiles_h * a.tiles_w > 0x7fffffffLL) return MT4_EUNSUPPORTED;
+    a.ntiles = B * a.tiles_h * a.tiles_w;
     return ds ? launch<64, true>(a, (hipStream_t)stream) : launch<256, false>(a, (hipStream_t)stream);
 }
 
@@ -457,6 +551,7 @@
     a.tiles_h = cdiv(H, TH); a.tiles_w = cdiv(W, TW);
     a.nt = 1;
     if ((long long)B * a.tiles_h * a.tiles_w > 0x7fffffffLL) return MT4_EUNSUPPORTED;
+    a.ntiles = B * a.tiles_h * a.tiles_w;
     return launch<256, false, true>(a, (hipStream_t)stream);
 }
 
diff --git a/computervision_codes_amd/csrc/igemm_conv.hip b/computervision_codes_amd/csrc/igemm_conv.hip
--- a/computervision_codes_amd/csrc/igemm_conv.hip
+++ b/computervision_codes_amd/csrc/igemm_conv.hip
@@ -2,40 +2,6 @@
 #include <cstdlib>
 
 typedef __bf16 bf16x8_t __attribute__((ext_vector_type(8)));
-typedef unsigned v4u __attribute__((ext_vector_type(4)));
-
-__device__ __forceinline__ v4u make_srd(const void* p, unsigned bytes) {
-    const unsigned long long u = (unsigned long long)p;
-    v4u r;
-    r.x = __builtin_amdgcn_readfirstlane((unsigned)u);
-    r.y = __builtin_amdgcn_readfirstlane((unsigned)(u >> 32) & 0xffffu);
-    r.z = __builtin_amdgcn_readfirstlane(bytes);
-    r.w = 0x00020000u;
-    return r;
-}
-
-template <int N, int STRIDE>
-__device__ __forceinline__ void lds_dma16_group(v4u srd, const unsigned (&voff)[N], unsigned soff, unsigned lds_addr) {
-    unsigned keep;
-    if constexpr (N == 1) {
-        asm volatile("s_mov_b32 %0, m0\n\ts_mov_b32 m0, %4\n\ts_nop 0\n\tbuffer_load_dwordx4 %1, %2, %3 offen lds\n\ts_mov_b32 m0, %0"
-                     : "=&s"(keep) : "v"(voff[0]), "s"(srd), "s"(soff), "s"(lds_addr) : "memory");
-    } else if constexpr (N == 2) {
-        asm volatile("s_mov_b32 %0, m0\n\ts_mov_b32 m0, %5\n\ts_nop 0\n\tbuffer_load_dwordx4 %1, %3, %4 offen lds\n\t"
-                     "s_add_u32 m0, m0, %6\n\ts_nop 0\n\tbuffer_load_dwordx4 %2, %3, %4 offen lds\n\ts_mov_b32 m0, %0"
-                     : "=&s"(keep) : "v"(voff[0]), "v"(voff[1]), "s"(srd), "s"(soff), "s"(lds_addr), "n"(STRIDE) : "memory", "scc");
-    } else {
-        static_assert(N == 4, "1, 2 or 4 pieces");
-        asm volatile("s_mov_b32 %0, m0\n\ts_mov_b32 m0, %7\n\ts_nop 0\n\tbuffer_load_dwordx4 %1, %5, %6 offen lds\n\t"
-                     "s_add_u32 m0, m0, %8\n\ts_nop 0\n\tbuffer_load_dwordx4 %2, %5, %6 offen lds\n\t"
-                     "s_add_u32 m0, m0, %8\n\ts_nop 0\n\tbuffer_load_dwordx4 %3, %5, %6 offen lds\n\t"
-                     "s_add_u32 m0, m0, %8\n\ts_nop 0\n\tbuffer_load_dwordx4 %4, %5, %6 offen lds\n\ts_mov_b32 m0, %0"
-                     : "=&s"(keep) : "v"(voff[0]), "v"(voff[1]), "v"(voff[2]), "v"(voff[3]), "s"(srd), "s"(soff), "s"(lds_addr),
-                       "n"(STRIDE)
-                     : "memory", "scc");
-    }
-}
-
 __device__ __forceinline__ void lds_dma16(v4u srd, unsigned voff, unsigned lds_addr) {
     unsigned keep;
     asm volatile(
diff --git a/computervision_codes_amd/csrc/mt4_common.h b/computervision_codes_amd/csrc/mt4_common.h
--- a/computervision_codes_amd/csrc/mt4_common.h
+++ b/computervision_codes_amd/csrc/mt4_common.h
@@ -71,6 +71,40 @@
     }
 }
 
+typedef unsigned v4u __attribute__((ext_vector_type(4)));
+
+__device__ __forceinline__ v4u make_srd(const void* p, unsigned bytes) {
+    const unsigned long long u = (unsigned long long)p;
+    v4u r;
+    r.x = __builtin_amdgcn_readfirstlane((unsigned)u);
+    r.y = __builtin_amdgcn_readfirstlane((unsigned)(u >> 32) & 0xffffu);
+    r.z = __builtin_amdgcn_readfirstlane(bytes);
+    r.w = 0x00020000u;
+    return r;
+}
+
+template <int N, int STRIDE>
+__device__ __forceinline__ void lds_dma16_group(v4u srd, const unsigned (&voff)[N], unsigned soff, unsigned lds_addr) {
+    unsigned keep;
+    if constexpr (N == 1) {
+        asm volatile("s_mov_b32 %0, m0\n\ts_mov_b32 m0, %4\n\ts_nop 0\n\tbuffer_load_dwordx4 %1, %2, %3 offen lds\n\ts_mov_b32 m0, %0"
+                     : "=&s"(keep) : "v"(voff[0]), "s"(srd), "s"(soff), "s"(lds_addr) : "memory");
+    } else if constexpr (N == 2) {
+        asm volatile("s_mov_b32 %0, m0\n\ts_mov_b32 m0, %5\n\ts_nop 0\n\tbuffer_load_dwordx4 %1, %3, %4 offen lds\n\t"
+                     "s_add_u32 m0, m0, %6\n\ts_nop 0\n\tbuffer_load_dwordx4 %2, %3, %4 offen lds\n\ts_mov_b32 m0, %0"
+                     : "=&s"(keep) : "v"(voff[0]), "v"(voff[1]), "s"(srd), "s"(soff), "s"(lds_addr), "n"(STRIDE) : "memory", "scc");
+    } else {
+        static_assert(N == 4, "1, 2 or 4 pieces");
+        asm volatile("s_mov_b32 %0, m0\n\ts_mov_b32 m0, %7\n\ts_nop 0\n\tbuffer_load_dwordx4 %1, %5, %6 offen lds\n\t"
+                     "s_add_u32 m0, m0, %8\n\ts_nop 0\n\tbuffer_load_dwordx4 %2, %5, %6 offen lds\n\t"
+                     "s_add_u32 m0, m0, %8\n\ts_nop 0\n\tbuffer_load_dwordx4 %3, %5, %6 offen lds\n\t"
+                     "s_add_u32 m0, m0, %8\n\ts_nop 0\n\tbuffer_load_dwordx4 %4, %5, %6 offen lds\n\ts_mov_b32 m0, %0"
+                     : "=&s"(keep) : "v"(voff[0]), "v"(voff[1]), "v"(voff[2]), "v"(voff[3]), "s"(srd), "s"(soff), "s"(lds_addr),
+                       "n"(STRIDE)
+                     : "memory", "scc");
+    }
+}
+
 static inline int cdiv(int a, int b) { return (a + b - 1) / b; }
 
 #define MT4_RAISE_LDS(fn)                                                                                                   \
```

Result: no change. 97560, median of 6 (+0.5%).
